# mll-lab-nu/TStar

Hardware: AMD Instinct MI355X
Metric: candidate frames scored/sec (whole node) + sec/video to 8 keyframes, 1h@1fps (higher is better)
Workload: dtype f32 held exactly as 3 bf16 terms per operand: every GEMM and vision-attention operand (activations, weights, Q, K, V, softmax probabilities) = three round-to-nearest bf16 terms carrying all 24 significand bits; the 6 partial products with i + j <= 2 (each exact) on v_mfma_f32_32x32x16_bf16, f32 accu

## Files before the change

include/tstar_hip.h:

```cpp
#ifndef TSTAR_HIP_H
#define TSTAR_HIP_H

#include <stddef.h>
#include <stdint.h>

#ifdef __cplusplus
extern "C" {
#endif

#define TSTAR_OK 0
#define TSTAR_ERR_ARG 1
#define TSTAR_ERR_HIP 2
#define TSTAR_ERR_STATE 3

#define TSTAR_OWL_NPATCH 576
#define TSTAR_OWL_QDIM 512
#define TSTAR_OWL_TEXT_LEN 16
#define TSTAR_OWL_MAX_QUERIES 32
#define TSTAR_OWL_MAX_SETS 64

const char* tstar_last_error(void);
int tstar_abi_version(void);
size_t tstar_owl_vision_blob_floats(void);
size_t tstar_owl_text_blob_floats(void);

typedef struct tstar_owl tstar_owl;

#define TSTAR_WEIGHTS_F32 0
#define TSTAR_WEIGHTS_BF16 1
#define TSTAR_WEIGHTS_BF16_EXACT 3
#define TSTAR_WEIGHTS_F32X3 4
int tstar_owl_create(tstar_owl** out, const float* h_vision_blob, size_t n_vision,
                     const float* h_text_blob, size_t n_text, const float* h_norm_lut, int max_batch,
                     int weights_mode);
int tstar_owl_create_ex(tstar_owl** out, int image_size, int patch_size, const float* h_vision_blob, size_t n_vision,
                        const float* h_text_blob, size_t n_text, const float* h_norm_lut, int max_batch, int weights_mode);
size_t tstar_owl_vision_blob_floats_ex(int image_size, int patch_size);
int tstar_owl_create_in(tstar_owl** out, int input_h, int input_w, int patch_size, const float* h_vision_blob, size_t n_vision,
                        const float* h_text_blob, size_t n_text, const float* h_norm_lut, int max_batch, int weights_mode);
size_t tstar_owl_vision_blob_floats_in(int input_h, int input_w, int patch_size);
#define TSTAR_OWL_FAMILY_OWLVIT 0
#define TSTAR_OWL_FAMILY_OWLV2 1
int tstar_owl_create_family(tstar_owl** out, int family, int input_h, int input_w, int patch_size, const float* h_vision_blob,
                            size_t n_vision, const float* h_text_blob, size_t n_text, const float* h_norm, int max_batch,
                            int weights_mode);
size_t tstar_owl_vision_blob_floats_family(int family, int input_h, int input_w, int patch_size);
int tstar_owl_num_patches(tstar_owl* h);
int tstar_owl_destroy(tstar_owl* h);

int tstar_owl_set_queries(tstar_owl* h, int query_set, const int32_t* h_input_ids, const int32_t* h_attention_mask,
                          const double* h_class_weight, int Q, void* stream);
int tstar_owl_set_queries_many(tstar_owl* h, int n_sets, const int32_t* h_sets, const int32_t* h_Q, const int32_t* h_ids,
                               const int32_t* h_am, const double* h_w, void* stream);
int tstar_owl_set_query_embeds(tstar_owl* h, int query_set, const float* h_query_embeds, const uint8_t* h_query_mask,
                               const double* h_class_weight, int Q, void* stream);
int tstar_owl_set_class_weights(tstar_owl* h, int query_set, const double* h_class_weight, int Q, void* stream);
int tstar_owl_get_query_embeds(tstar_owl* h, int query_set, float* h_out, int Q, void* stream);

int tstar_owl_score(tstar_owl* h, const uint8_t* d_images, int B, int H, int W, int grid_rows, int grid_cols,
                    const int32_t* h_image_query_set, float* d_scores, int32_t* d_labels, float* d_boxes_xyxy, double* d_cell_conf,
                    uint32_t* d_cell_mask, int32_t* d_n_kept, float* d_logits, float* d_boxes_cxcywh, void* stream);
#define TSTAR_OWL_LANES 2
#define TSTAR_OWL_AUX_BATCH 4
int tstar_owl_score_lane(tstar_owl* h, int lane, const uint8_t* d_images, int B, int H, int W, int grid_rows, int grid_cols,
                         const int32_t* h_image_query_set, float* d_scores, int32_t* d_labels, float* d_boxes_xyxy,
                         double* d_cell_conf, uint32_t* d_cell_mask, int32_t* d_n_kept, float* d_logits,
                         float* d_boxes_cxcywh, void* stream);

int tstar_owl_score_lane_obj(tstar_owl* h, int lane, const uint8_t* d_images, int B, int H, int W, int grid_rows, int grid_cols,
                             const int32_t* h_image_query_set, float* d_scores, int32_t* d_labels, float* d_boxes_xyxy,
                             double* d_cell_conf, uint32_t* d_cell_mask, int32_t* d_n_kept, float* d_logits,
                             float* d_boxes_cxcywh, float* d_objectness, void* stream);

int tstar_owlv2_set_axis_weights(tstar_owl* h, int S, int out, const double* gw, int n);
int tstar_owlv2_preprocess_plan(int H, int W, int out_h, int out_w, int* plan10);
int tstar_owlv2_axis_window(int S, int out, int tile, int k, int radius, int* lo_n2);
int tstar_owlv2_axis_tables(int S, int out, int32_t* i0, int32_t* i1, double* t, double* gw, int gw_cap);
int tstar_owlv2_last_preprocess_form(tstar_owl* h, int lane);

int tstar_owl_debug_preprocess(tstar_owl* h, const uint8_t* d_images, int B, int H, int W,
                               uint8_t* d_out_u8 , float* d_out_patches ,
                               void* stream);

int tstar_owl_debug_heads(tstar_owl* h, const float* d_feats, const float* d_cls, const float* d_boxh, int B, int H, int W,
                          const int32_t* h_image_query_set, float* d_scores, int32_t* d_labels, float* d_boxes_xyxy, float* d_logits,
                          float* d_boxes_cxcywh, const float* d_obj_hidden, float* d_objectness, void* stream);
int tstar_owl_debug_merge(tstar_owl* h, float* d_x, int B, int write_cls, float* d_feats, void* stream);
int tstar_owl_debug_embed(tstar_owl* h, const float* d_patches, int B, int stage, float* d_x, void* stream);
int tstar_owl_debug_text(tstar_owl* h, const int32_t* h_ids, const int32_t* h_am, int Q, int stage, float* h_out, void* stream);
int tstar_cell_reduce(const float* d_scores, const int32_t* d_labels, const float* d_boxes_xyxy, const double* h_weights, int n_sets,
                      const int32_t* h_image_set, int B, int np, int W, int H, int grid_rows, int grid_cols, float thr,
                      double* d_cell_conf, uint32_t* d_cell_mask, int32_t* d_n_kept, void* stream);

int tstar_owl_embed_image_queries(tstar_owl* h, const uint8_t* d_images, int n, int H, int W, float* h_embeds, int32_t* h_best,
                                  float* h_boxes_cxcywh, int32_t* h_n_selected, int32_t* h_status, void* stream);
int tstar_image_query_select(const float* d_cls, const float* d_boxes_cxcywh, int n, int np, float* h_embeds, int32_t* h_best,
                             float* h_boxes_cxcywh, int32_t* h_n_selected, int32_t* h_status, void* stream);

typedef struct tstar_yolo tstar_yolo;
int tstar_yolo_create(tstar_yolo** out, const float* h_blob, size_t n_blob, const int32_t* h_ops, int n_ops, int op_words,
                      const int32_t* h_bufs, int n_bufs, const int32_t* h_guides, int n_guides, const int32_t* h_levels,
                      int n_levels, int input_buf, int max_batch);
int tstar_yolo_destroy(tstar_yolo* h);
int tstar_yolo_num_anchors(tstar_yolo* h);
int tstar_yolo_set_text_feats(tstar_yolo* h, int query_set, const float* h_text, const double* h_class_weight, int Q, void* stream);
int tstar_yolo_set_class_weights(tstar_yolo* h, int query_set, const double* h_class_weight, int Q, void* stream);
int tstar_yolo_detect(tstar_yolo* h, const uint8_t* d_images, int B, int H, int W, int grid_rows, int grid_cols,
                      const int32_t* h_image_query_set, float score_threshold, int max_dets, float* d_det_scores,
                      int32_t* d_det_labels, float* d_det_boxes, int32_t* d_n_det, double* d_cell_conf, uint32_t* d_cell_mask,
                      float* d_dense_scores, float* d_dense_boxes, void* stream);
int tstar_yolo_postprocess(tstar_yolo* h, const float* const* d_level_embed, const float* const* d_level_dfl, int n_levels, int B, int H,
                           int W, int grid_rows, int grid_cols, const int32_t* h_image_query_set, float score_threshold, int max_dets,
                           float* d_det_scores, int32_t* d_det_labels, float* d_det_boxes, int32_t* d_n_det, double* d_cell_conf,
                           uint32_t* d_cell_mask, float* d_dense_scores, float* d_dense_boxes, void* stream);

#define TSTAR_YOLO_FORM_TILE64 0
#define TSTAR_YOLO_FORM_TILE128 1
#define TSTAR_YOLO_FORM_WIDE 2
#define TSTAR_YOLO_FORM_SW8 3
#define TSTAR_YOLO_FORM_SW4 4
#define TSTAR_YOLO_FORM_HALO_A16 5
#define TSTAR_YOLO_FORM_HALO_A8 6
#define TSTAR_YOLO_FORM_HALO_B16 7
#define TSTAR_YOLO_FORM_HALO_B8 8
#define TSTAR_YOLO_FORM_DIRECT 9
int tstar_yolo_buffer_copy(tstar_yolo* h, int buf, float* d_data, int B, int to_buffer, void* stream);
int tstar_yolo_run_ops(tstar_yolo* h, int B, const int32_t* h_image_query_set, int32_t* h_forms, void* stream);
int tstar_yolo_conv_plan(int cin, int src_ld, int src_off, int H, int W, int cout, int dst_ld, int dst_off, int ks, int stride, int mode, int B,
                         int max_batch, int env_policy, int* plan3);

int tstar_frames_to_grid(const uint8_t* d_video, int N, int H, int W, const int32_t* d_frame_idx,
                         int grid_rows, int grid_cols, uint8_t* d_grid, int nv12, void* stream);
int tstar_frames_resize(const uint8_t* d_video, int N, int H, int W, const int32_t* d_frame_idx, int n,
                        int out_w, int out_h, uint8_t* d_out, int nv12, void* stream);
int tstar_i420_to_nv12(const uint8_t* d_i420, int n, int H, int W, uint8_t* d_nv12, void* stream);
int tstar_jpeg_probe(const uint8_t* data, size_t len, int32_t* info5);
size_t tstar_jpeg_frame_end(const uint8_t* data, size_t len, size_t pos);
int tstar_jpeg_sizes(int W, int H, int ncomp, int hs, int vs, size_t* out2);
int tstar_jpeg_threads(int asked);
int tstar_jpeg_entropy_batch(const uint8_t* const* datas, const size_t* lens, int n, int W, int H, int ncomp, int hs, int vs,
                             int16_t* coef, uint16_t* quant, int threads, int32_t* status);
int tstar_jpeg_reconstruct_host(const int16_t* coef, const uint16_t* quant, int n, int W, int H, int ncomp, int hs, int vs,
                                uint8_t* rgb, int threads);
int tstar_jpeg_reconstruct(const int16_t* d_coef, const uint16_t* d_quant, int n, int W, int H, int ncomp, int hs, int vs,
                           uint8_t* d_planes, uint8_t* d_rgb, void* stream);
int tstar_nv12_to_rgb(const uint8_t* d_video, int N, int H, int W, const int32_t* d_frame_idx, int n,
                      uint8_t* d_out, void* stream);

typedef struct tstar_searcher tstar_searcher;
int tstar_searcher_create(tstar_searcher** out, int n_frames, double init_score, double init_p);
int tstar_searcher_destroy(tstar_searcher* s);
int tstar_searcher_apply_grid(tstar_searcher* s, const int32_t* h_secs, const double* d_conf, int n,
                              int* h_n_visited, int32_t* h_vis_x, double* h_vis_y, void* stream);
int tstar_searcher_window_spread(tstar_searcher* s, const int32_t* h_secs, const double* h_conf, int n, int window,
                                 void* stream);
int tstar_searcher_visited(tstar_searcher* s, int* h_n_visited, int32_t* h_vis_x, double* h_vis_y, void* stream);
int tstar_searcher_set_spline(tstar_searcher* s, const double* h_t, const double* h_c, int n_knots, int k, void* stream);
int tstar_searcher_sampler_prep(tstar_searcher* s, int num, double add, int* h_fallback, void* stream);
int tstar_searcher_pop_prep(tstar_searcher* s, int* h_nnz, double* h_sum, void* stream);
int tstar_searcher_draw(tstar_searcher* s, const double* h_x, int k, int32_t* h_idx, void* stream);
int tstar_searcher_exclude(tstar_searcher* s, const int32_t* h_found, int m, void* stream);
int tstar_searcher_set_scores(tstar_searcher* s, const int32_t* h_secs, const double* h_vals, int m, void* stream);
int tstar_searcher_read_state(tstar_searcher* s, double* h_out, void* stream);
int tstar_searcher_write(tstar_searcher* s, int which, const double* h_in, void* stream);
int tstar_searcher_read(tstar_searcher* s, int which, double* h_out, void* stream);

#define TSTAR_COMM_ID_BYTES 128
typedef struct tstar_comm tstar_comm;
int tstar_comm_available(void);
int tstar_comm_unique_id(void* h_id );
int tstar_comm_create(tstar_comm** out, const void* h_id, int world, int rank);
int tstar_comm_destroy(tstar_comm* c);
int tstar_allgather_i32(tstar_comm* c, const int32_t* d_send, int32_t* d_recv, int count, void* stream);

int tstar_topk_seconds(const double* d_P, int N, int clip_start, int clip_end, int k, int32_t* h_out, void* stream);

int tstar_ssim_pairwise(const uint8_t* d_gt, int G, const uint8_t* d_pred, int P, int H, int W,
                        const float* h_window, double* d_out, void* stream);

int tstar_draw_boxes(uint8_t* d_images, int B, int H, int W, const float* d_boxes_xyxy, const float* d_scores, void* stream);
int tstar_draw_boxes_np(uint8_t* d_images, int B, int H, int W, const float* d_boxes_xyxy, const float* d_scores, int np,
                        void* stream);

int tstar_gemm_f32(const float* d_A, const float* d_W, float* d_C, const float* d_bias, const float* d_residual,
                   int M, int N, int K, int act, void* stream);
int tstar_gemm_f32_cfg(const float* d_A, const float* d_W, float* d_C, const float* d_bias, const float* d_residual,
                       int M, int N, int K, int act, int tile_cfg, void* stream);
int tstar_gemm_bf16w(const float* d_A, const float* d_W, float* d_C, const float* d_bias, const float* d_residual,
                     int M, int N, int K, int act, int tile_cfg, void* stream);
int tstar_gemm_bf16w2(const float* d_A, const float* d_W, float* d_C, const float* d_bias, const float* d_residual,
                      int M, int N, int K, int act, int tile_cfg, void* stream);
int tstar_gemm_bf16w_pre(const float* d_A, const void* d_Wb, float* d_C, const float* d_bias, const float* d_residual,
                         int M, int N, int K, int act, int a_terms, int tile_cfg, void* stream);
int tstar_gemm_f32x3(const float* d_A, const float* d_W, float* d_C, const float* d_bias, const float* d_residual,
                     int M, int N, int K, int act, int tile_cfg, void* stream);
int tstar_pack_f32x3(const float* d_W, void* d_Wp, int N, int K, void* stream);
int tstar_gemm_f32x3_pre(const float* d_A, const void* d_Wp, float* d_C, const float* d_bias, const float* d_residual,
                         int M, int N, int K, int act, int tile_cfg, void* stream);
int tstar_gemm_plan(int weights_mode, int M, int N, int ldc, int patch_np, int tile_cfg, int has_packed_w2, int* plan4);
int tstar_gemm_patch_embed(const float* d_A, const float* d_W, float* d_X, const float* d_pos, int B, int np, int N, int K,
                           int weights_mode, int tile_cfg, void* stream);
int tstar_ingest_plan(int op, int nv12, int H, int W, int n, int ow, int oh, int out_aligned4, int video_aligned4, int generic,
                      int nv12_lds, int grid_px, int* plan6);
int tstar_layernorm_f32(const float* d_x, float* d_y, const float* d_w, const float* d_b, int rows, int D, void* stream);
int tstar_attention_f32(const float* d_qkv, float* d_out, int B, int T, int heads, int mode,
                        const uint8_t* d_key_mask, void* stream);

int tstar_attention_split(const float* d_qkv, float* d_out, int B, int T, int heads, void* stream);
int tstar_attention_x3(const float* d_qkv, float* d_out, int B, int T, int heads, void* stream);

int tstar_prof_enable(int on);
int tstar_prof_read(int category, long long* launches, double* total_ms, double* total_flops);
int tstar_prof_read_bytes(int category, double* total_bytes);
int tstar_prof_read_totals(int category, long long* launches_all, double* flops_all);
int tstar_prof_mark(int which, void* stream);

#ifdef __cplusplus
}
#endif
#endif
```

tstar_amd/_lib.py:

```python
from __future__ import annotations

import ctypes as C
import os

_HERE = os.path.dirname(os.path.abspath(__file__))
LIB_PATH = os.path.join(_HERE, "libtstar_hip.so")


class TStarHipError(RuntimeError):
    pass


_vp, _i, _sz = C.c_void_p, C.c_int, C.c_size_t
_fp = C.POINTER(C.c_float)
SIGNATURES = {
    "tstar_last_error": (C.c_char_p, []),
    "tstar_abi_version": (_i, []),
    "tstar_owl_vision_blob_floats": (_sz, []),
    "tstar_owl_text_blob_floats": (_sz, []),
    "tstar_owl_create": (_i, [C.POINTER(_vp), _vp, _sz, _vp, _sz, _vp, _i, _i]),
    "tstar_owl_create_ex": (_i, [C.POINTER(_vp), _i, _i, _vp, _sz, _vp, _sz, _vp, _i, _i]),
    "tstar_owl_vision_blob_floats_ex": (_sz, [_i, _i]),
    "tstar_owl_create_in": (_i, [C.POINTER(_vp), _i, _i, _i, _vp, _sz, _vp, _sz, _vp, _i, _i]),
    "tstar_owl_vision_blob_floats_in": (_sz, [_i, _i, _i]),
    "tstar_owl_create_family": (_i, [C.POINTER(_vp), _i, _i, _i, _i, _vp, _sz, _vp, _sz, _vp, _i, _i]),
    "tstar_owl_vision_blob_floats_family": (_sz, [_i, _i, _i, _i]),
    "tstar_owl_score_lane_obj": (_i, [_vp, _i, _vp, _i, _i, _i, _i, _i, _vp, _vp, _vp, _vp, _vp, _vp, _vp, _vp, _vp, _vp, _vp]),
    "tstar_owlv2_set_axis_weights": (_i, [_vp, _i, _i, _vp, _i]),
    "tstar_owlv2_preprocess_plan": (_i, [_i, _i, _i, _i, C.POINTER(_i)]),
    "tstar_owlv2_axis_window": (_i, [_i, _i, _i, _i, _i, C.POINTER(_i)]),
    "tstar_owlv2_axis_tables": (_i, [_i, _i, _vp, _vp, _vp, _vp, _i]),
    "tstar_owlv2_last_preprocess_form": (_i, [_vp, _i]),
    "tstar_owl_num_patches": (_i, [_vp]),
    "tstar_owl_destroy": (_i, [_vp]),
    "tstar_owl_set_queries": (_i, [_vp, _i, _vp, _vp, _vp, _i, _vp]),
    "tstar_owl_set_queries_many": (_i, [_vp, _i, _vp, _vp, _vp, _vp, _vp, _vp]),
    "tstar_owl_set_query_embeds": (_i, [_vp, _i, _vp, _vp, _vp, _i, _vp]),
    "tstar_owl_set_class_weights": (_i, [_vp, _i, _vp, _i, _vp]),
    "tstar_owl_get_query_embeds": (_i, [_vp, _i, _vp, _i, _vp]),
    "tstar_owl_score": (_i, [_vp, _vp, _i, _i, _i, _i, _i, _vp, _vp, _vp, _vp, _vp, _vp, _vp, _vp, _vp, _vp]),
    "tstar_owl_score_lane": (_i, [_vp, _i, _vp, _i, _i, _i, _i, _i, _vp, _vp, _vp, _vp, _vp, _vp, _vp, _vp, _vp, _vp]),
    "tstar_owl_debug_preprocess": (_i, [_vp, _vp, _i, _i, _i, _vp, _vp, _vp]),
    "tstar_owl_debug_heads": (_i, [_vp, _vp, _vp, _vp, _i, _i, _i, _vp, _vp, _vp, _vp, _vp, _vp, _vp, _vp, _vp]),
    "tstar_owl_debug_merge": (_i, [_vp, _vp, _i, _i, _vp, _vp]),
    "tstar_owl_debug_embed": (_i, [_vp, _vp, _i, _i, _vp, _vp]),
    "tstar_owl_debug_text": (_i, [_vp, _vp, _vp, _i, _i, _vp, _vp]),
    "tstar_cell_reduce": (_i, [_vp, _vp, _vp, _vp, _i, _vp, _i, _i, _i, _i, _i, _i, C.c_float, _vp, _vp, _vp, _vp]),
    "tstar_owl_embed_image_queries": (_i, [_vp, _vp, _i, _i, _i, _vp, _vp, _vp, _vp, _vp, _vp]),
    "tstar_image_query_select": (_i, [_vp, _vp, _i, _i, _vp, _vp, _vp, _vp, _vp, _vp]),
    "tstar_yolo_create": (_i, [C.POINTER(_vp), _vp, _sz, _vp, _i, _i, _vp, _i, _vp, _i, _vp, _i, _i, _i]),
    "tstar_yolo_destroy": (_i, [_vp]),
    "tstar_yolo_num_anchors": (_i, [_vp]),
    "tstar_yolo_set_text_feats": (_i, [_vp, _i, _vp, _vp, _i, _vp]),
    "tstar_yolo_set_class_weights": (_i, [_vp, _i, _vp, _i, _vp]),
    "tstar_yolo_detect": (_i, [_vp, _vp, _i, _i, _i, _i, _i, _vp, C.c_float, _i, _vp, _vp, _vp, _vp, _vp, _vp, _vp, _vp, _vp]),
    "tstar_yolo_postprocess": (_i, [_vp, _vp, _vp, _i, _i, _i, _i, _i, _i, _vp, C.c_float, _i, _vp, _vp, _vp, _vp, _vp, _vp, _vp, _vp, _vp]),
    "tstar_yolo_buffer_copy": (_i, [_vp, _i, _vp, _i, _i, _vp]),
    "tstar_yolo_run_ops": (_i, [_vp, _i, _vp, _vp, _vp]),
    "tstar_yolo_conv_plan": (_i, [_i] * 14 + [C.POINTER(_i)]),
    "tstar_frames_to_grid": (_i, [_vp, _i, _i, _i, _vp, _i, _i, _vp, _i, _vp]),
    "tstar_frames_resize": (_i, [_vp, _i, _i, _i, _vp, _i, _i, _i, _vp, _i, _vp]),
    "tstar_i420_to_nv12": (_i, [_vp, _i, _i, _i, _vp, _vp]),
    "tstar_nv12_to_rgb": (_i, [_vp, _i, _i, _i, _vp, _i, _vp, _vp]),
    "tstar_jpeg_probe": (_i, [_vp, _sz, _vp]),
    "tstar_jpeg_frame_end": (_sz, [_vp, _sz, _sz]),
    "tstar_jpeg_sizes": (_i, [_i, _i, _i, _i, _i, _vp]),
    "tstar_jpeg_threads": (_i, [_i]),
    "tstar_jpeg_entropy_batch": (_i, [_vp, _vp, _i, _i, _i, _i, _i, _i, _vp, _vp, _i, _vp]),
    "tstar_jpeg_reconstruct_host": (_i, [_vp, _vp, _i, _i, _i, _i, _i, _i, _vp, _i]),
    "tstar_jpeg_reconstruct": (_i, [_vp, _vp, _i, _i, _i, _i, _i, _i, _vp, _vp, _vp]),
    "tstar_searcher_create": (_i, [C.POINTER(_vp), _i, C.c_double, C.c_double]),
    "tstar_searcher_destroy": (_i, [_vp]),
    "tstar_searcher_apply_grid": (_i, [_vp, _vp, _vp, _i, _vp, _vp, _vp, _vp]),
    "tstar_searcher_set_spline": (_i, [_vp, _vp, _vp, _i, _i, _vp]),
    "tstar_searcher_sampler_prep": (_i, [_vp, _i, C.c_double, _vp, _vp]),
    "tstar_searcher_pop_prep": (_i, [_vp, _vp, _vp, _vp]),
    "tstar_searcher_window_spread": (_i, [_vp, _vp, _vp, _i, _i, _vp]),
    "tstar_searcher_visited": (_i, [_vp, _vp, _vp, _vp, _vp]),
    "tstar_searcher_write": (_i, [_vp, _i, _vp, _vp]),
    "tstar_searcher_draw": (_i, [_vp, _vp, _i, _vp, _vp]),
    "tstar_searcher_exclude": (_i, [_vp, _vp, _i, _vp]),
    "tstar_searcher_set_scores": (_i, [_vp, _vp, _vp, _i, _vp]),
    "tstar_searcher_read_state": (_i, [_vp, _vp, _vp]),
    "tstar_searcher_read": (_i, [_vp, _i, _vp, _vp]),
    "tstar_comm_available": (_i, []),
    "tstar_comm_unique_id": (_i, [_vp]),
    "tstar_comm_create": (_i, [C.POINTER(_vp), _vp, _i, _i]),
    "tstar_comm_destroy": (_i, [_vp]),
    "tstar_allgather_i32": (_i, [_vp, _vp, _vp, _i, _vp]),
    "tstar_topk_seconds": (_i, [_vp, _i, _i, _i, _i, _vp, _vp]),
    "tstar_ssim_pairwise": (_i, [_vp, _i, _vp, _i, _i, _i, _vp, _vp, _vp]),
    "tstar_gemm_f32": (_i, [_vp, _vp, _vp, _vp, _vp, _i, _i, _i, _i, _vp]),
    "tstar_gemm_f32_cfg": (_i, [_vp, _vp, _vp, _vp, _vp, _i, _i, _i, _i, _i, _vp]),
    "tstar_gemm_bf16w": (_i, [_vp, _vp, _vp, _vp, _vp, _i, _i, _i, _i, _i, _vp]),
    "tstar_gemm_bf16w2": (_i, [_vp, _vp, _vp, _vp, _vp, _i, _i, _i, _i, _i, _vp]),
    "tstar_gemm_bf16w_pre": (_i, [_vp, _vp, _vp, _vp, _vp, _i, _i, _i, _i, _i, _i, _vp]),
    "tstar_gemm_f32x3": (_i, [_vp, _vp, _vp, _vp, _vp, _i, _i, _i, _i, _i, _vp]),
    "tstar_pack_f32x3": (_i, [_vp, _vp, _i, _i, _vp]),
    "tstar_gemm_f32x3_pre": (_i, [_vp, _vp, _vp, _vp, _vp, _i, _i, _i, _i, _i, _vp]),
    "tstar_gemm_plan": (_i, [_i, _i, _i, _i, _i, _i, _i, C.POINTER(_i)]),
    "tstar_gemm_patch_embed": (_i, [_vp, _vp, _vp, _vp, _i, _i, _i, _i, _i, _i, _vp]),
    "tstar_ingest_plan": (_i, [_i] * 12 + [C.POINTER(_i)]),
    "tstar_layernorm_f32": (_i, [_vp, _vp, _vp, _vp, _i, _i, _vp]),
    "tstar_draw_boxes": (_i, [_vp, _i, _i, _i, _vp, _vp, _vp]),
    "tstar_draw_boxes_np": (_i, [_vp, _i, _i, _i, _vp, _vp, _i, _vp]),
    "tstar_attention_split": (_i, [_vp, _vp, _i, _i, _i, _vp]),
    "tstar_attention_x3": (_i, [_vp, _vp, _i, _i, _i, _vp]),
    "tstar_attention_f32": (_i, [_vp, _vp, _i, _i, _i, _i, _vp, _vp]),
    "tstar_prof_enable": (_i, [_i]),
    "tstar_prof_read": (_i, [_i, _vp, _vp, _vp]),
    "tstar_prof_read_bytes": (_i, [_i, _vp]),
    "tstar_prof_read_totals": (_i, [_i, _vp, _vp]),
    "tstar_prof_mark": (_i, [_i, _vp]),
}

_lib = None


def load() -> C.CDLL:
    global _lib
    if _lib is not None:
        return _lib
    if not os.path.isfile(LIB_PATH):
        raise TStarHipError(
            f"{LIB_PATH} is missing: build it with `python -m tstar_amd.build` "
            "(hipcc --offload-arch=gfx950). tstar_amd has no CPU fallback.")
    import torch
    lib = C.CDLL(LIB_PATH)
    for name, (res, args) in SIGNATURES.items():
        fn = getattr(lib, name)
        fn.restype = res
        fn.argtypes = args
    _lib = lib
    return lib


def check(rc: int, what: str = "") -> None:
    if rc != 0:
        msg = load().tstar_last_error()
        raise TStarHipError(f"{what or 'tstar_hip'} failed (code {rc}): {msg.decode() if msg else ''}")


def ptr(t) -> int:
    if t is None:
        return None
    if hasattr(t, "data_ptr"):
        return t.data_ptr()
    return t.ctypes.data


def stream_ptr():
    import torch
    return torch.cuda.current_stream().cuda_stream
```

tstar_amd/csrc/attention_x3.h:

```cpp
#pragma once
#include <hip/hip_runtime.h>
#include <math.h>
#include <utility>

namespace tstar {
namespace ax3 {

typedef __bf16 bf16x8 __attribute__((ext_vector_type(8)));
typedef __bf16 bf16x2 __attribute__((ext_vector_type(2)));
typedef float f32x2 __attribute__((ext_vector_type(2)));
typedef float f32x4 __attribute__((ext_vector_type(4)));
typedef float f32x16 __attribute__((ext_vector_type(16)));
typedef unsigned int u32x4 __attribute__((ext_vector_type(4)));
typedef unsigned int u32x2 __attribute__((ext_vector_type(2)));

constexpr int HD = 64, KB = 32;
constexpr int VPITCH = 80;
constexpr int KP = KB * 128, VP = HD * VPITCH;
constexpr int KBUF = 3 * KP, VBUF = 3 * VP, NKB = 2, NVB = 3;
constexpr int LDS_BYTES = NKB * KBUF + NVB * VBUF;

#define AX3_FENCE() __builtin_amdgcn_sched_barrier(0)

__device__ __forceinline__ void split2_rn3(float x0, float x1, unsigned (&o)[3]) {
#pragma unroll
    for (int k = 0; k < 3; ++k) {
        f32x2 x; x[0] = x0; x[1] = x1;
        const unsigned hb = __builtin_bit_cast(unsigned, __builtin_convertvector(x, bf16x2));
        o[k] = hb;
        if (k < 2) {
            x0 = x0 - __uint_as_float(hb << 16);
            x1 = x1 - __uint_as_float(hb & 0xFFFF0000u);
        }
    }
}
__device__ __forceinline__ float xhalf_max(float x) {
    const auto r = __builtin_amdgcn_permlane32_swap(__float_as_uint(x), __float_as_uint(x), false, false);
    return fmaxf(__uint_as_float(r[0]), __uint_as_float(r[1]));
}
__device__ __forceinline__ float xhalf_sum(float x) {
    const auto r = __builtin_amdgcn_permlane32_swap(__float_as_uint(x), __float_as_uint(x), false, false);
    return __uint_as_float(r[0]) + __uint_as_float(r[1]);
}

__device__ __forceinline__ int k_off(int key, int chunk) { return key * 128 + ((chunk ^ ((key >> 1) & 7)) << 4); }
__device__ __forceinline__ int v_off(int d, int chunk) { return d * VPITCH + (chunk << 4); }
__device__ __forceinline__ int v_keypos(int k) { const int g = k >> 2; const int gp = (g & 4) | ((g & 1) << 1) | ((g >> 1) & 1); return (gp * 4 + (k & 3)) * 2; }

__device__ __forceinline__ f32x16 mfma(const bf16x8 a, const u32x4 b, const f32x16 c) {
    return __builtin_amdgcn_mfma_f32_32x32x16_bf16(a, __builtin_bit_cast(bf16x8, b), c, 0, 0, 0);
}

template <bool PLANES>
__global__ __launch_bounds__(256, 2) void attention_x3_kernel(const float* __restrict__ qkv, const char* __restrict__ planes,
                                                              float* __restrict__ out, int T, int heads, int qtiles) {
    extern __shared__ __attribute__((aligned(16))) char smem[];
    char* const kbuf = smem;
    char* const vbuf = smem + NKB * KBUF;

    const int D = heads * HD, D3 = 3 * D;
    int bid = blockIdx.x;
    const int qt = bid % qtiles; bid /= qtiles;
    const int head = bid % heads;
    const int b = bid / heads;

    const int t = threadIdx.x, lane = t & 63, wave = __builtin_amdgcn_readfirstlane(t >> 6);
    const int l31 = lane & 31, h = lane >> 5;
    const size_t rowbase = (size_t)b * T;

    const int q = qt * 128 + wave * 32 + l31;
    const int qc = q < T ? q : T - 1;
    const bool wave_active = (qt * 128 + wave * 32) < T;

    u32x4 qp[3][4];
    {
        const float* src = qkv + (rowbase + qc) * D3 + head * HD + 8 * h;
        const float sc = 0.125f * 1.44269504088896340736f;
#pragma unroll
        for (int s = 0; s < 4; ++s) {
            const f32x4 a = *reinterpret_cast<const f32x4*>(src + 16 * s) * sc;
            const f32x4 c = *reinterpret_cast<const f32x4*>(src + 16 * s + 4) * sc;
            unsigned o0[3], o1[3], o2[3], o3[3];
            split2_rn3(a[0], a[1], o0); split2_rn3(a[2], a[3], o1); split2_rn3(c[0], c[1], o2); split2_rn3(c[2], c[3], o3);
#pragma unroll
            for (int k = 0; k < 3; ++k) { qp[k][s][0] = o0[k]; qp[k][s][1] = o1[k]; qp[k][s][2] = o2[k]; qp[k][s][3] = o3[k]; }
        }
    }

    const int kc4 = t & 15, kr = t >> 4;
    const int vkp = t & 15, vdq = t >> 4;
    const __amdgpu_buffer_rsrc_t kv_rsrc =
        __builtin_amdgcn_make_buffer_rsrc(const_cast<float*>(qkv + rowbase * D3), 0, (int)((size_t)T * D3 * 4), 0x00020000);
    int kvo[2], vvo[2];
#pragma unroll
    for (int i = 0; i < 2; ++i) {
        kvo[i] = ((kr + 16 * i) * D3 + D + head * HD + kc4 * 4) * 4;
        vvo[i] = ((2 * vkp + i) * D3 + 2 * D + head * HD + vdq * 4) * 4;
    }
    const int kwr0 = k_off(kr, kc4 >> 1) + (kc4 & 1) * 8, kwr1 = k_off(kr + 16, kc4 >> 1) + (kc4 & 1) * 8;
    int vwr[4];
#pragma unroll
    for (int e = 0; e < 4; ++e) {
        const int pos = v_keypos(2 * vkp);
        vwr[e] = v_off(4 * vdq + e, pos >> 4) + (pos & 15);
    }

    const int R0 = b * T;
    const int kt0 = R0 >> 5;
    const bool tail_key = !PLANES && (T % KB) == 1;
    const int nkb = PLANES ? ((R0 + T - 1) >> 5) - kt0 + 1 : (tail_key ? T / KB : (T + KB - 1) / KB);

    f32x4 rk[2], rv[2];
    auto gload = [&](int kb) __attribute__((always_inline)) {
        const int so = (kb < nkb ? kb : nkb) * (KB * 4) * D3;
#pragma unroll
        for (int i = 0; i < 2; ++i) {
            rk[i] = __builtin_bit_cast(f32x4, __builtin_amdgcn_raw_buffer_load_b128(kv_rsrc, kvo[i], so, 0));
            rv[i] = __builtin_bit_cast(f32x4, __builtin_amdgcn_raw_buffer_load_b128(kv_rsrc, vvo[i], so, 0));
        }
    };
    unsigned ksp[2][3];
    auto stage_piece = [&](auto P, char* kdst, char* vdst) __attribute__((always_inline)) {
        constexpr int p = decltype(P)::value;
        if constexpr (p < 4) {
            constexpr int i = p >> 1, hf = p & 1;
            split2_rn3(rk[i][2 * hf], rk[i][2 * hf + 1], ksp[hf]);
            if constexpr (hf == 1) {
#pragma unroll
                for (int k = 0; k < 3; ++k) {
                    u32x2 v; v[0] = ksp[0][k]; v[1] = ksp[1][k];
                    *reinterpret_cast<u32x2*>(kdst + k * KP + (i == 0 ? kwr0 : kwr1)) = v;
                }
            }
        } else {
            constexpr int e = p - 4;
            unsigned o[3];
            split2_rn3(rv[0][e], rv[1][e], o);
#pragma unroll
            for (int k = 0; k < 3; ++k) *reinterpret_cast<unsigned*>(vdst + k * VP + vwr[e]) = o[k];
        }
    };
    auto stage_all = [&](int kb) __attribute__((always_inline)) {
        char* kd = kbuf + (kb & 1) * KBUF;
        char* vd = vbuf + (kb % NVB) * VBUF;
// ... 250 lines not shown
            }
        }
        sx = xhalf_sum(sx);
        const float mn = fmaxf(m_run, sx);
        const float al = __builtin_amdgcn_exp2f(m_run - mn);
        const float p = __builtin_amdgcn_exp2f(sx - mn);
        l_run = l_run * al + p;
        m_run = mn;
#pragma unroll
        for (int g4 = 0; g4 < 4; ++g4) {
            const f32x4 v0 = *reinterpret_cast<const f32x4*>(qkv + ro + 2 * D + 8 * g4 + 4 * h);
            const f32x4 v1 = *reinterpret_cast<const f32x4*>(qkv + ro + 2 * D + 32 + 8 * g4 + 4 * h);
#pragma unroll
            for (int e = 0; e < 4; ++e) {
                o0[g4 * 4 + e] = o0[g4 * 4 + e] * al + p * v0[e];
                o1[g4 * 4 + e] = o1[g4 * 4 + e] * al + p * v1[e];
            }
        }
    }

    if (q < T) {
        const float inv = 1.0f / l_run;
        float* op = out + (rowbase + q) * D + head * HD + 4 * h;
#pragma unroll
        for (int g4 = 0; g4 < 4; ++g4) {
            f32x4 a, c;
#pragma unroll
            for (int e = 0; e < 4; ++e) { a[e] = o0[g4 * 4 + e] * inv; c[e] = o1[g4 * 4 + e] * inv; }
            *reinterpret_cast<f32x4*>(op + 8 * g4) = a;
            *reinterpret_cast<f32x4*>(op + 32 + 8 * g4) = c;
        }
    }
}

}

inline size_t kv_planes_bytes(int rows, int heads) { return (size_t)((rows + 31) / 32) * heads * (size_t)(ax3::KBUF + ax3::VBUF); }

#ifdef TSTAR_ATTN_X3_LAB
namespace ax3 {
__global__ __launch_bounds__(256) void kv_planes_kernel(const float* __restrict__ qkv, char* __restrict__ planes, int rows, int heads) {
    const int D = heads * HD, D3 = 3 * D;
    const size_t gid = (size_t)blockIdx.x * 256 + threadIdx.x;
    const int dq = (int)(gid % 16), head = (int)((gid / 16) % heads);
    const size_t rp = gid / (16 * (size_t)heads);
    const int row = (int)(rp * 2);
    if (row >= ((rows + 31) / 32) * 32) return;
    const int kt = row >> 5, key = row & 31;
    char* tile = planes + ((size_t)kt * heads + head) * (size_t)(KBUF + VBUF);
    f32x4 kx[2], vx[2];
#pragma unroll
    for (int i = 0; i < 2; ++i) {
        if (row + i < rows) {
            kx[i] = *reinterpret_cast<const f32x4*>(qkv + (size_t)(row + i) * D3 + D + head * HD + dq * 4);
            vx[i] = *reinterpret_cast<const f32x4*>(qkv + (size_t)(row + i) * D3 + 2 * D + head * HD + dq * 4);
        } else {
            kx[i] = f32x4{0.f, 0.f, 0.f, 0.f};
            vx[i] = f32x4{0.f, 0.f, 0.f, 0.f};
        }
    }
#pragma unroll
    for (int i = 0; i < 2; ++i) {
        unsigned o0[3], o1[3];
        split2_rn3(kx[i][0], kx[i][1], o0);
        split2_rn3(kx[i][2], kx[i][3], o1);
#pragma unroll
        for (int k = 0; k < 3; ++k) {
            u32x2 v; v[0] = o0[k]; v[1] = o1[k];
            *reinterpret_cast<u32x2*>(tile + k * KP + k_off(key + i, dq >> 1) + (dq & 1) * 8) = v;
        }
    }
    const int pos = v_keypos(key);
#pragma unroll
    for (int e = 0; e < 4; ++e) {
        unsigned o[3];
        split2_rn3(vx[0][e], vx[1][e], o);
#pragma unroll
        for (int k = 0; k < 3; ++k) *reinterpret_cast<unsigned*>(tile + KBUF + k * VP + v_off(4 * dq + e, pos >> 4) + (pos & 15)) = o[k];
    }
}
}
#endif

inline int attention_x3_launch(const float* qkv, float* out, int B, int T, int heads, hipStream_t s, const char* planes = nullptr) {
    const int qtiles = (T + 127) / 128;
#ifdef TSTAR_ATTN_X3_LAB
    static bool attr[2] = {false, false};
    if (planes) {
        if (!attr[1]) {
            const hipError_t e = hipFuncSetAttribute(reinterpret_cast<const void*>(ax3::attention_x3_kernel<true>), hipFuncAttributeMaxDynamicSharedMemorySize, ax3::LDS_BYTES);
            if (e != hipSuccess) return (int)e;
            attr[1] = true;
        }
        hipLaunchKernelGGL(ax3::attention_x3_kernel<true>, dim3(B * heads * qtiles), dim3(256), ax3::LDS_BYTES, s, qkv, planes, out, T, heads, qtiles);
        return (int)hipGetLastError();
    }
    if (!attr[0]) {
        const hipError_t e = hipFuncSetAttribute(reinterpret_cast<const void*>(ax3::attention_x3_kernel<false>), hipFuncAttributeMaxDynamicSharedMemorySize, ax3::LDS_BYTES);
        if (e != hipSuccess) return (int)e;
        attr[0] = true;
    }
#endif
    if (planes) return (int)hipErrorInvalidValue;
    hipLaunchKernelGGL(ax3::attention_x3_kernel<false>, dim3(B * heads * qtiles), dim3(256), ax3::LDS_BYTES, s, qkv, planes, out, T, heads, qtiles);
    return (int)hipGetLastError();
}

#ifdef TSTAR_ATTN_X3_LAB
inline int kv_planes_launch(const float* qkv, char* planes, int rows, int heads, hipStream_t s) {
    const size_t n = (size_t)((rows + 31) / 32) * 16 * 16 * heads;
    hipLaunchKernelGGL(ax3::kv_planes_kernel, dim3((unsigned)((n + 255) / 256)), dim3(256), 0, s, qkv, planes, rows, heads);
    return (int)hipGetLastError();
}
#endif

}
```

tstar_amd/csrc/attention_x3.hip:

```cpp
#include "common.h"
#include "kernels.h"
#include "prof.h"
#include "attention_x3.h"

namespace tstar {

int attention_x3(const float* qkv, float* out, int B, int T, int heads, hipStream_t s) {
    TSTAR_REQUIRE(B > 0 && T > 0 && heads > 0, "attention_x3: empty problem");
    TSTAR_REQUIRE(((size_t)T + 32) * 3 * heads * 64 * 4 < (1ull << 31), "attention_x3: one image's qkv rows (plus one key tile of look-ahead) must stay below 2 GiB");
    if (int rc = ensure_dyn_lds(reinterpret_cast<const void*>(ax3::attention_x3_kernel<false>), ax3::LDS_BYTES)) return rc;
    const bool prof = prof_enabled();
    if (prof) prof_start(PROF_ATTN, s, 4.0 * B * heads * (double)T * T * 64);
    const int rc = attention_x3_launch(qkv, out, B, T, heads, s);
    if (prof) prof_stop(PROF_ATTN, s);
    TSTAR_HIP_CHECK((hipError_t)rc);
    return TSTAR_OK;
}

}
```

tstar_amd/csrc/capi.hip:

```cpp
#include "../../include/tstar_hip.h"
#include "common.h"
#include "heads.h"
#include "image_query.h"
#include "ingest.h"
#include "jpeg_host.h"
#include "kernels.h"
#include "owl_weights.h"
#include "preprocess_v2.h"
#include <math.h>
#include <map>
#include <mutex>
#include <set>
#include <string.h>
#include <unordered_map>
#include <vector>

namespace tstar {
static thread_local std::string g_err;
void set_error(const std::string& msg) { g_err = msg; }

int ensure_dyn_lds(const void* kernel, int bytes) {
    static std::mutex mu;
    static std::set<std::pair<const void*, int>> done;
    int dev = 0;
// ... 230 lines not shown
static int preprocess_chunk(tstar_owl* h, tstar_owl::Lane& L, const uint8_t* d_images, int B, int H, int W, uint8_t* out_u8,
                            float* out_patches, hipStream_t s) {
    if (h->geom.family == TSTAR_OWL_FAMILY_OWLV2) {
        TSTAR_REQUIRE(!out_u8, "tstar_owl_debug_preprocess: an OWLv2 handle has no u8 stage (d_out_u8 must be NULL)");
        return preprocess_chunk_v2(h, L, d_images, B, H, W, out_patches, s);
    }
    ResampleTable *th, *tv;
    const OwlGeom& G = h->geom;
    RC(get_table(h, W, G.in_w, &th, s));
    RC(get_table(h, H, G.in_h, &tv, s));
    const size_t need = (size_t)B * H * G.in_w * 3;
    if (need > L.tmp_u8_bytes) {
        TSTAR_HIP_CHECK(hipStreamSynchronize(s));
        if (L.tmp_u8) TSTAR_HIP_CHECK(hipFree(L.tmp_u8));
        L.tmp_u8 = nullptr; L.tmp_u8_bytes = 0;
        TSTAR_HIP_CHECK(hipMalloc(&L.tmp_u8, need));
        L.tmp_u8_bytes = need;
    }
    RC(resample_h_u8(d_images, L.tmp_u8, B, H, W, *th, s));
    RC(resample_v_normalize_patchify(L.tmp_u8, out_patches, out_u8, B, H, G.in_w, *tv, h->d_lut, G.patch, s));
    return TSTAR_OK;
}

static hipError_t alloc_lane(tstar_owl::Lane& L, int cap, const OwlGeom& g) {
    const size_t mp = lane_rows(cap, g);
    hipError_t e = hipSuccess;
    auto alloc = [&](float** p, size_t n) { if (e == hipSuccess) { e = hipMalloc(p, n * sizeof(float)); if (e == hipSuccess) e = hipMemset(*p, 0, n * sizeof(float)); } };
    alloc(&L.x, mp * V_D); alloc(&L.xn, mp * V_D); alloc(&L.qkv, mp * 3 * V_D); alloc(&L.att, mp * V_D); alloc(&L.hid, mp * V_FF);
    if (e == hipSuccess) L.cap = cap;
    return e;
}
static void free_lane(tstar_owl::Lane& L) {
    void* ptrs[] = {L.x, L.xn, L.qkv, L.att, L.hid, L.tmp_u8, L.d_image_set, L.d_minmax};
    for (void* p : ptrs) if (p) (void)hipFree(p);
    L = tstar_owl::Lane{};
}

#define CHECK_SET(set, fn) TSTAR_REQUIRE((set) >= 0 && (set) < TSTAR_OWL_MAX_SETS, fn ": query_set must be in 0..63")

static int check_image_sets(const tstar_owl* h, const int32_t* h_image_query_set, int B, int* q_uniform) {
    int qu = -1;
    for (int b = 0; b < B; ++b) {
        const int set = h_image_query_set ? h_image_query_set[b] : 0;
        CHECK_SET(set, "tstar_owl_score");
        if (h->Q[set] == 0) { set_error("tstar_owl_score: no queries installed in the requested query set (call tstar_owl_set_queries first)"); return TSTAR_ERR_STATE; }
        qu = (b == 0 || qu == h->Q[set]) ? h->Q[set] : 0;
    }
    *q_uniform = qu;
    return TSTAR_OK;
}

static int stage_image_sets(tstar_owl::Lane& L, const int32_t* h_image_query_set, int B, hipStream_t s) {
    if (B > L.image_set_cap) {
        TSTAR_HIP_CHECK(hipStreamSynchronize(s));
        if (L.d_image_set) TSTAR_HIP_CHECK(hipFree(L.d_image_set));
        L.d_image_set = nullptr; L.image_set_cap = 0;
        TSTAR_HIP_CHECK(hipMalloc(&L.d_image_set, (size_t)B * sizeof(int)));
        L.image_set_cap = B;
    }
    TSTAR_HIP_CHECK(hipMemcpyAsync(L.d_image_set, h_image_query_set, (size_t)B * sizeof(int), hipMemcpyHostToDevice, s));
    return TSTAR_OK;
}

static void box_scale(const OwlGeom& G, int H, int W, float* sx, float* sy) {
    const bool v2 = G.family == TSTAR_OWL_FAMILY_OWLV2;
    *sx = (float)(v2 ? (H > W ? H : W) : W);
    *sy = (float)(v2 ? (H > W ? H : W) : H);
}

static DetectRowsArgs detect_args(const tstar_owl* h) {
    DetectRowsArgs a{};
    a.qn = h->qn; a.qmask = h->qmask; a.setQ = h->d_setQ;
    a.shift_w = h->vw.shift_w; a.shift_b = h->vw.shift_b; a.scale_w = h->vw.scale_w; a.scale_b = h->vw.scale_b;
    a.box2_w = h->vw.box2_w; a.box2_b = h->vw.box2_b; a.box_bias = h->vw.box_bias;
    return a;
}

struct OwlHeadTensors {
    float* feats;
    float* cls;
    float* bh1;
    float* bh2;
};
static int owl_forward_heads(tstar_owl* h, tstar_owl::Lane& L, const uint8_t* d_images, int Bc, int H, int W, OwlHeadTensors* t, hipStream_t s) {
    const OwlGeom& G = h->geom;
    const int NP = G.np, NTOK = G.ntok, PK = G.patch_k;
    const int M = Bc * NTOK, MP = Bc * NP;
    RC(preprocess_chunk(h, L, d_images, Bc, H, W, nullptr, L.hid, s));
    GemmArgs pg = mk_gemm(h, L.hid, h->vw.patch_w, L.x, nullptr, nullptr, MP, V_D, PK, PK, V_D, ACT_NONE);
    pg.pos = h->vw.pos_emb; pg.patch_np = NP;
    RC(gemm_f32(pg, s));
    RC(write_cls_rows(L.x, h->vw.class_emb, h->vw.pos_emb, Bc, NTOK, V_D, s));
    RC(layernorm_f32(L.x, L.x, h->vw.pre_ln_w, h->vw.pre_ln_b, M, V_D, s));
    RC(run_encoder(h, L, h->vw.layers, V_LAYERS, Bc, NTOK, V_D, V_FF, V_HEADS, 0, nullptr, s));
    t->feats = L.xn; t->cls = L.att; t->bh1 = L.qkv; t->bh2 = L.hid;
    RC(merge_cls_ln(L.x, t->feats, h->vw.post_ln_w, h->vw.post_ln_b, h->vw.det_ln_w, h->vw.det_ln_b, Bc, NTOK, V_D, s));
    RC(gemm_f32(mk_gemm(h, t->feats, h->vw.cls_w, t->cls, h->vw.cls_b, nullptr, MP, PROJ, V_D, V_D, PROJ, ACT_NONE), s));
    RC(gemm_f32(mk_gemm(h, t->feats, h->vw.box0_w, t->bh1, h->vw.box0_b, nullptr, MP, V_D, V_D, V_D, V_D, ACT_GELU), s));
    RC(gemm_f32(mk_gemm(h, t->bh1, h->vw.box1_w, t->bh2, h->vw.box1_b, nullptr, MP, V_D, V_D, V_D, V_D, ACT_GELU), s));
    return TSTAR_OK;
}

extern "C" {

const char* tstar_last_error(void) { return g_err.c_str(); }
int tstar_abi_version(void) { return 3; }
size_t tstar_owl_vision_blob_floats(void) { return vision_floats(OwlGeom{}); }
size_t tstar_owl_text_blob_floats(void) { return text_floats(); }
size_t tstar_owl_vision_blob_floats_ex(int image_size, int patch_size) {
    OwlGeom g;
    if (!owl_geom(image_size, patch_size, &g)) { set_error("tstar_owl_vision_blob_floats_ex: unsupported geometry (image 768, patch 32 or 16)"); return 0; }
    return vision_floats(g);
}
size_t tstar_owl_vision_blob_floats_in(int input_h, int input_w, int patch_size) {
    OwlGeom g;
    if (!owl_geom_input(input_h, input_w, patch_size, &g)) {
        set_error("tstar_owl_vision_blob_floats_in: unsupported input size (patch 32 or 16; each side a positive multiple of the patch size; at most 3600 patches)");
        return 0;
    }
    return vision_floats(g);
}
size_t tstar_owl_vision_blob_floats_family(int family, int input_h, int input_w, int patch_size) {
    OwlGeom g;
    if (!owl_geom_family(family, input_h, input_w, patch_size, &g)) {
        set_error("tstar_owl_vision_blob_floats_family: unsupported family / input size (family 0: patch 32 or 16; family 1 (OWLv2): patch 16; each "
                  "side a positive multiple of the patch size; at most 3600 patches)");
        return 0;
    }
    return vision_floats(g);
}
int tstar_owl_num_patches(tstar_owl* h) {
    if (!h) { set_error("tstar_owl_num_patches: null handle"); return -1; }
    return h->geom.np;
}

static int make_bf16_copies(tstar_owl* h, int mode) {
    struct Mat { const float* w; int n, k; };
    std::vector<Mat> mats;
    mats.push_back({h->vw.patch_w, V_D, h->geom.patch_k});
    auto layer = [&](const LayerW& l, int d, int ff) {
        mats.push_back({l.qkv_w, 3 * d, d}); mats.push_back({l.out_w, d, d});
        mats.push_back({l.fc1_w, ff, d}); mats.push_back({l.fc2_w, d, ff});
    };
    for (int i = 0; i < V_LAYERS; ++i) layer(h->vw.layers[i], V_D, V_FF);
    mats.push_back({h->vw.cls_w, PROJ, V_D});
    mats.push_back({h->vw.box0_w, V_D, V_D});
    mats.push_back({h->vw.box1_w, V_D, V_D});
    if (h->vw.obj0_w) { mats.push_back({h->vw.obj0_w, V_D, V_D}); mats.push_back({h->vw.obj1_w, V_D, V_D}); }
    if (h->has_text) {
        for (int i = 0; i < T_LAYERS; ++i) layer(h->tw.layers[i], T_D, T_FF);
        mats.push_back({h->tw.text_proj, PROJ, T_D});
    }
    for (auto& m : mats) {
        const size_t n = (size_t)m.n * m.k;
        int rc;
        if (mode == TSTAR_WEIGHTS_F32X3) {
            void* p = nullptr;
            TSTAR_HIP_CHECK(hipMalloc(&p, n * 6));
            h->wp[m.w] = p;
            rc = pack_weights_x3(m.w, p, m.n, m.k, 0);
        } else {
            __bf16* p = nullptr;
            TSTAR_HIP_CHECK(hipMalloc(&p, n * sizeof(__bf16)));
            h->wb[m.w] = p;
            rc = convert_f32_to_bf16(m.w, p, nullptr, n, 0);
            static const bool w2v_off = getenv("TSTAR_W2V_OFF") != nullptr;
            if (!rc && mode == TSTAR_WEIGHTS_BF16 && m.n == 768 && m.k % 32 == 0 && !w2v_off) {
                void* q = nullptr;
                TSTAR_HIP_CHECK(hipMalloc(&q, n * sizeof(__bf16)));
                h->wq[m.w] = q;
                rc = pack_weights_w2(p, q, m.n, m.k, 0);
            }
        }
        if (rc) return rc;
    }
    TSTAR_HIP_CHECK(hipDeviceSynchronize());
    h->weights_mode = mode;
    return TSTAR_OK;
}

// ... 209 lines not shown
        TSTAR_HIP_CHECK(hipMalloc(&h->d_kmask, (size_t)cap * T_LEN));
        h->seq_cap = cap;
    }
    std::vector<int> eos(total);
    std::vector<uint8_t> km((size_t)total * T_LEN), qm(total);
    for (int q = 0; q < total; ++q) {
        int best = 0;
        for (int t = 0; t < T_LEN; ++t) {
            if (h_ids[q * T_LEN + t] > h_ids[q * T_LEN + best]) best = t;
            km[(size_t)q * T_LEN + t] = h_am[q * T_LEN + t] != 0;
        }
        eos[q] = best;
        qm[q] = h_ids[q * T_LEN] > 0;
    }
    int i0 = 0, q0 = 0;
    while (i0 < n_sets) {
        int i1 = i0, nseq = 0;
        while (i1 < n_sets && nseq + h_Q[i1] <= cap) nseq += h_Q[i1++];
        const int M = nseq * T_LEN;
        TSTAR_HIP_CHECK(hipMemcpyAsync(h->d_ids, h_ids + (size_t)q0 * T_LEN, (size_t)M * sizeof(int), hipMemcpyHostToDevice, s));
        TSTAR_HIP_CHECK(hipMemcpyAsync(h->d_eos, eos.data() + q0, nseq * sizeof(int), hipMemcpyHostToDevice, s));
        TSTAR_HIP_CHECK(hipMemcpyAsync(h->d_kmask, km.data() + (size_t)q0 * T_LEN, M, hipMemcpyHostToDevice, s));
        hipLaunchKernelGGL(embed_tokens_kernel, dim3(M), dim3(128), 0, s, h->d_ids, h->tw.tok_emb, h->tw.tpos_emb, L.x, T_LEN, T_D);
        TSTAR_HIP_CHECK(hipGetLastError());
        RC(run_encoder(h, L, h->tw.layers, T_LAYERS, nseq, T_LEN, T_D, T_FF, T_HEADS, 1, h->d_kmask, s));
        RC(layernorm_f32(L.x, L.xn, h->tw.final_ln_w, h->tw.final_ln_b, M, T_D, s));
        hipLaunchKernelGGL(gather_rows_kernel, dim3(nseq), dim3(128), 0, s, L.xn, h->d_eos, L.att, T_LEN, T_D);
        TSTAR_HIP_CHECK(hipGetLastError());
        RC(gemm_f32(mk_text_gemm(h, L.att, h->tw.text_proj, L.hid, nullptr, nullptr, nseq, PROJ, T_D, T_D, PROJ, ACT_NONE), s));
        int off = 0;
        for (int i = i0; i < i1; ++i) {
            const int set = h_sets[i], Q = h_Q[i];
            const size_t qo = (size_t)set * TSTAR_OWL_MAX_QUERIES;
            hipLaunchKernelGGL(l2norm_rows_kernel, dim3(Q), dim3(64), 0, s, L.hid + (size_t)off * PROJ, h->q_raw + qo * PROJ, 0.0f);
            hipLaunchKernelGGL(l2norm_rows_kernel, dim3(Q), dim3(64), 0, s, h->q_raw + qo * PROJ, h->qn + qo * PROJ, 1e-6f);
            TSTAR_HIP_CHECK(hipGetLastError());
            TSTAR_HIP_CHECK(hipMemcpyAsync(h->qmask + qo, qm.data() + q0 + off, Q, hipMemcpyHostToDevice, s));
            TSTAR_HIP_CHECK(hipMemcpyAsync(h->qweight + qo, h_w + q0 + off, Q * sizeof(double), hipMemcpyHostToDevice, s));
            h->Q[set] = Q;
            off += Q;
        }
        TSTAR_HIP_CHECK(hipStreamSynchronize(s));
        q0 += nseq;
        i0 = i1;
    }
    TSTAR_HIP_CHECK(hipMemcpyAsync(h->d_setQ, h->Q, sizeof(h->Q), hipMemcpyHostToDevice, s));
    TSTAR_HIP_CHECK(hipStreamSynchronize(s));
    return TSTAR_OK;
}

int tstar_owl_set_query_embeds(tstar_owl* h, int query_set, const float* h_qe, const uint8_t* h_mask, const double* h_w,
                               int Q, void* stream) {
    TSTAR_REQUIRE(h && h_qe && h_mask && h_w, "tstar_owl_set_query_embeds: null argument");
    CHECK_SET(query_set, "tstar_owl_set_query_embeds");
    TSTAR_REQUIRE(Q >= 1 && Q <= TSTAR_OWL_MAX_QUERIES, "tstar_owl_set_query_embeds: Q must be in 1..32");
    hipStream_t s = (hipStream_t)stream;
    TSTAR_HIP_CHECK(hipMemcpyAsync(h->q_raw + (size_t)query_set * TSTAR_OWL_MAX_QUERIES * PROJ, h_qe,
                                   (size_t)Q * PROJ * sizeof(float), hipMemcpyHostToDevice, s));
    return finish_queries(h, query_set, h_mask, h_w, Q, s);
}

int tstar_owl_set_class_weights(tstar_owl* h, int query_set, const double* h_w, int Q, void* stream) {
    TSTAR_REQUIRE(h && h_w, "tstar_owl_set_class_weights: null argument");
    CHECK_SET(query_set, "tstar_owl_set_class_weights");
    TSTAR_REQUIRE(Q == h->Q[query_set] && Q >= 1, "tstar_owl_set_class_weights: Q does not match the installed queries");
    hipStream_t s = (hipStream_t)stream;
    TSTAR_HIP_CHECK(hipMemcpyAsync(h->qweight + (size_t)query_set * TSTAR_OWL_MAX_QUERIES, h_w, Q * sizeof(double),
                                   hipMemcpyHostToDevice, s));
    TSTAR_HIP_CHECK(hipStreamSynchronize(s));
    return TSTAR_OK;
}

int tstar_owl_get_query_embeds(tstar_owl* h, int query_set, float* h_out, int Q, void* stream) {
    TSTAR_REQUIRE(h && h_out, "tstar_owl_get_query_embeds: null argument");
    CHECK_SET(query_set, "tstar_owl_get_query_embeds");
    TSTAR_REQUIRE(Q == h->Q[query_set], "tstar_owl_get_query_embeds: Q does not match the installed queries");
    hipStream_t s = (hipStream_t)stream;
    TSTAR_HIP_CHECK(hipMemcpyAsync(h_out, h->q_raw + (size_t)query_set * TSTAR_OWL_MAX_QUERIES * PROJ,
                                   (size_t)Q * PROJ * sizeof(float), hipMemcpyDeviceToHost, s));
    TSTAR_HIP_CHECK(hipStreamSynchronize(s));
    return TSTAR_OK;
}

int tstar_owl_score(tstar_owl* h, const uint8_t* d_images, int B, int H, int W, int grid_rows, int grid_cols,
                    const int32_t* h_image_query_set, float* d_scores, int32_t* d_labels, float* d_boxes_xyxy, double* d_cell_conf,
                    uint32_t* d_cell_mask, int32_t* d_n_kept, float* d_logits, float* d_boxes_cxcywh, void* stream) {
    return tstar_owl_score_lane(h, 0, d_images, B, H, W, grid_rows, grid_cols, h_image_query_set, d_scores, d_labels, d_boxes_xyxy, d_cell_conf,
                                d_cell_mask, d_n_kept, d_logits, d_boxes_cxcywh, stream);
}

int tstar_owl_score_lane(tstar_owl* h, int lane, const uint8_t* d_images, int B, int H, int W, int grid_rows, int grid_cols,
                         const int32_t* h_image_query_set, float* d_scores, int32_t* d_labels, float* d_boxes_xyxy, double* d_cell_conf,
                         uint32_t* d_cell_mask, int32_t* d_n_kept, float* d_logits, float* d_boxes_cxcywh, void* stream) {
    return tstar_owl_score_lane_obj(h, lane, d_images, B, H, W, grid_rows, grid_cols, h_image_query_set, d_scores, d_labels, d_boxes_xyxy, d_cell_conf,
                                    d_cell_mask, d_n_kept, d_logits, d_boxes_cxcywh, nullptr, stream);
}

int tstar_owl_score_lane_obj(tstar_owl* h, int lane, const uint8_t* d_images, int B, int H, int W, int grid_rows, int grid_cols,
                             const int32_t* h_image_query_set, float* d_scores, int32_t* d_labels, float* d_boxes_xyxy, double* d_cell_conf,
                             uint32_t* d_cell_mask, int32_t* d_n_kept, float* d_logits, float* d_boxes_cxcywh, float* d_objectness, void* stream) {
    TSTAR_REQUIRE(h && d_images && d_scores && d_labels && d_boxes_xyxy && d_cell_conf && d_cell_mask,
                  "tstar_owl_score: null argument");
    TSTAR_REQUIRE(lane >= 0 && lane < TSTAR_OWL_LANES, "tstar_owl_score_lane: lane must be 0 or 1");
    TSTAR_REQUIRE(B >= 1 && H >= 1 && W >= 1, "tstar_owl_score: empty batch or image");
    TSTAR_REQUIRE(grid_rows >= 1 && grid_cols >= 1, "tstar_owl_score: grid must be at least 1x1");
    if (!h->has_vision) { set_error("tstar_owl_score: handle was created without vision weights (text-only)"); return TSTAR_ERR_STATE; }
    TSTAR_REQUIRE(!d_objectness || h->geom.family == TSTAR_OWL_FAMILY_OWLV2, "tstar_owl_score_lane_obj: objectness needs an OWLv2 handle (OWL-ViT has no objectness head)");
    if (h->geom.family == TSTAR_OWL_FAMILY_OWLV2) {
        const Owlv2Plan vp = plan_owlv2_preprocess(H, W, h->geom.in_h, h->geom.in_w);
        if (vp.error) { set_error(vp.error); return TSTAR_ERR_ARG; }
    }
    hipStream_t s = (hipStream_t)stream;
    auto& L = h->lane[lane];
    if (lane != 0) {
        int need = B > TSTAR_OWL_AUX_BATCH ? B : TSTAR_OWL_AUX_BATCH;
        if (need > h->chunk_cap) need = h->chunk_cap;
        if (!L.x || L.cap < need) {
            if (L.x) { TSTAR_HIP_CHECK(hipDeviceSynchronize()); free_lane(L); }
            const hipError_t e = alloc_lane(L, need, h->geom);
            if (e != hipSuccess) {
                free_lane(L);
                set_error(std::string("tstar_owl_score_lane: workspace allocation failed: ") + hipGetErrorString(e));
                return TSTAR_ERR_HIP;
            }
            TSTAR_HIP_CHECK(hipDeviceSynchronize());
        }
    }
    int q_uniform = -1;
    RC(check_image_sets(h, h_image_query_set, B, &q_uniform));
    TSTAR_REQUIRE(!d_logits || q_uniform > 0, "tstar_owl_score: raw logits need the same query count for every image");
    if (h_image_query_set) RC(stage_image_sets(L, h_image_query_set, B, s));
    const int ncell = grid_rows * grid_cols;
    const OwlGeom& G = h->geom;
    const int NP = G.np;
    for (int b0 = 0; b0 < B; b0 += L.cap) {
        const int Bc = (B - b0) < L.cap ? (B - b0) : L.cap;
        const int MP = Bc * NP;
        OwlHeadTensors t;
        RC(owl_forward_heads(h, L, d_images + (size_t)b0 * H * W * 3, Bc, H, W, &t, s));
        float *feats = t.feats, *cls = t.cls, *bh1 = t.bh1, *bh2 = t.bh2;
        DetectRowsArgs a = detect_args(h);
        a.feats = feats; a.cls = cls; a.boxh = bh2;
        a.scores = d_scores + (size_t)b0 * NP;
        a.labels = d_labels + (size_t)b0 * NP;
        a.xyxy = d_boxes_xyxy + (size_t)b0 * NP * 4;
        a.logits = d_logits ? d_logits + (size_t)b0 * NP * q_uniform : nullptr;
        a.image_set = h_image_query_set ? L.d_image_set + b0 : nullptr;
        a.cxcywh = d_boxes_cxcywh ? d_boxes_cxcywh + (size_t)b0 * NP * 4 : nullptr;
        a.rows = MP; a.np = NP; a.Q = q_uniform;
        box_scale(G, H, W, &a.box_sx, &a.box_sy);
        RC(detect_rows(a, s));
        if (d_objectness) {
            RC(gemm_f32(mk_gemm(h, feats, h->vw.obj0_w, bh1, h->vw.obj0_b, nullptr, MP, V_D, V_D, V_D, V_D, ACT_GELU), s));
            RC(gemm_f32(mk_gemm(h, bh1, h->vw.obj1_w, bh2, h->vw.obj1_b, nullptr, MP, V_D, V_D, V_D, V_D, ACT_GELU), s));
            RC(row_dot768(bh2, h->vw.obj2_w, h->vw.obj2_b, d_objectness + (size_t)b0 * NP, MP, s));
        }
        RC(cell_reduce(a.scores, a.labels, a.xyxy, h->qweight, a.image_set, Bc, NP, W, H, grid_rows, grid_cols, 0.005f,
                       d_cell_conf + (size_t)b0 * ncell, d_cell_mask + (size_t)b0 * ncell,
                       d_n_kept ? d_n_kept + b0 : nullptr, s));
    }
    return TSTAR_OK;
}

int tstar_owl_debug_preprocess(tstar_owl* h, const uint8_t* d_images, int B, int H, int W, uint8_t* d_out_u8,
                               float* d_out_patches, void* stream) {
    TSTAR_REQUIRE(h && d_images && d_out_patches, "tstar_owl_debug_preprocess: null argument");
    TSTAR_REQUIRE(B >= 1 && B <= h->max_batch, "tstar_owl_debug_preprocess: B must be in 1..max_batch");
    if (!h->has_vision) { set_error("tstar_owl_debug_preprocess: handle was created without vision weights (text-only)"); return TSTAR_ERR_STATE; }
    return preprocess_chunk(h, h->lane[0], d_images, B, H, W, d_out_u8, d_out_patches, (hipStream_t)stream);
}

int tstar_owl_debug_heads(tstar_owl* h, const float* d_feats, const float* d_cls, const float* d_boxh, int B, int H, int W,
                          const int32_t* h_image_query_set, float* d_scores, int32_t* d_labels, float* d_boxes_xyxy, float* d_logits,
                          float* d_boxes_cxcywh, const float* d_obj_hidden, float* d_objectness, void* stream) {
    TSTAR_REQUIRE(h && d_feats && d_cls && d_boxh && d_scores && d_labels && d_boxes_xyxy, "tstar_owl_debug_heads: null argument");
    TSTAR_REQUIRE(B >= 1 && B <= h->max_batch, "tstar_owl_debug_heads: B must be in 1..max_batch");
    TSTAR_REQUIRE(H >= 1 && W >= 1, "tstar_owl_debug_heads: empty image");
    if (!h->has_vision) { set_error("tstar_owl_debug_heads: handle was created without vision weights (text-only)"); return TSTAR_ERR_STATE; }
    TSTAR_REQUIRE(!d_obj_hidden == !d_objectness, "tstar_owl_debug_heads: d_obj_hidden and d_objectness go together");
    TSTAR_REQUIRE(!d_objectness || h->geom.family == TSTAR_OWL_FAMILY_OWLV2, "tstar_owl_debug_heads: objectness needs an OWLv2 handle (OWL-ViT has no objectness head)");
    hipStream_t s = (hipStream_t)stream;
    auto& L = h->lane[0];
    int q_uniform = -1;
    RC(check_image_sets(h, h_image_query_set, B, &q_uniform));
    TSTAR_REQUIRE(!d_logits || q_uniform > 0, "tstar_owl_debug_heads: raw logits need the same query count for every image");
    if (h_image_query_set) RC(stage_image_sets(L, h_image_query_set, B, s));
    const int NP = h->geom.np;
    DetectRowsArgs a = detect_args(h);
    a.feats = d_feats; a.cls = d_cls; a.boxh = d_boxh;
    a.scores = d_scores; a.labels = d_labels; a.xyxy = d_boxes_xyxy; a.logits = d_logits; a.cxcywh = d_boxes_cxcywh;
    a.image_set = h_image_query_set ? L.d_image_set : nullptr;
    a.rows = B * NP; a.np = NP; a.Q = q_uniform;
    box_scale(h->geom, H, W, &a.box_sx, &a.box_sy);
    RC(detect_rows(a, s));
    if (d_objectness) RC(row_dot768(d_obj_hidden, h->vw.obj2_w, h->vw.obj2_b, d_objectness, B * NP, s));
    return TSTAR_OK;
}

int tstar_owl_debug_merge(tstar_owl* h, float* d_x, int B, int write_cls, float* d_feats, void* stream) {
    TSTAR_REQUIRE(h && d_x && d_feats, "tstar_owl_debug_merge: null argument");
    TSTAR_REQUIRE(B >= 1 && B <= h->max_batch, "tstar_owl_debug_merge: B must be in 1..max_batch");
    if (!h->has_vision) { set_error("tstar_owl_debug_merge: handle was created without vision weights (text-only)"); return TSTAR_ERR_STATE; }
    hipStream_t s = (hipStream_t)stream;
    if (write_cls) RC(write_cls_rows(d_x, h->vw.class_emb, h->vw.pos_emb, B, h->geom.ntok, V_D, s));
    return merge_cls_ln(d_x, d_feats, h->vw.post_ln_w, h->vw.post_ln_b, h->vw.det_ln_w, h->vw.det_ln_b, B, h->geom.ntok, V_D, s);
}

int tstar_owl_debug_embed(tstar_owl* h, const float* d_patches, int B, int stage, float* d_x, void* stream) {
    TSTAR_REQUIRE(h && d_patches && d_x, "tstar_owl_debug_embed: null argument");
    TSTAR_REQUIRE(stage == 0 || stage == 1, "tstar_owl_debug_embed: stage must be 0 (patch GEMM + class rows) or 1 (+ pre-LayerNorm)");
    if (!h->has_vision) { set_error("tstar_owl_debug_embed: handle was created without vision weights (text-only)"); return TSTAR_ERR_STATE; }
    auto& L = h->lane[0];
    TSTAR_REQUIRE(B >= 1 && B <= L.cap, "tstar_owl_debug_embed: B must be in 1..the images of one forward chunk (min(max_batch, chunk limit))");
    hipStream_t s = (hipStream_t)stream;
    const OwlGeom& G = h->geom;
    const int M = B * G.ntok;
    GemmArgs pg = mk_gemm(h, d_patches, h->vw.patch_w, L.x, nullptr, nullptr, B * G.np, V_D, G.patch_k, G.patch_k, V_D, ACT_NONE);
    pg.pos = h->vw.pos_emb; pg.patch_np = G.np;
    RC(gemm_f32(pg, s));
    RC(write_cls_rows(L.x, h->vw.class_emb, h->vw.pos_emb, B, G.ntok, V_D, s));
    if (stage == 1) RC(layernorm_f32(L.x, L.x, h->vw.pre_ln_w, h->vw.pre_ln_b, M, V_D, s));
    TSTAR_HIP_CHECK(hipMemcpyAsync(d_x, L.x, (size_t)M * V_D * sizeof(float), hipMemcpyDeviceToDevice, s));
    return TSTAR_OK;
}

int tstar_cell_reduce(const float* d_scores, const int32_t* d_labels, const float* d_boxes_xyxy, const double* h_weights, int n_sets,
                      const int32_t* h_image_set, int B, int np, int W, int H, int grid_rows, int grid_cols, float thr,
                      double* d_cell_conf, uint32_t* d_cell_mask, int32_t* d_n_kept, void* stream) {
    TSTAR_REQUIRE(d_scores && d_labels && d_boxes_xyxy && h_weights && d_cell_conf && d_cell_mask && d_n_kept, "tstar_cell_reduce: null argument");
    TSTAR_REQUIRE(B >= 1 && np >= 1 && W >= 1 && H >= 1, "tstar_cell_reduce: empty batch or image");
    TSTAR_REQUIRE(n_sets >= 1 && n_sets <= TSTAR_OWL_MAX_SETS, "tstar_cell_reduce: n_sets must be in 1..64");
    TSTAR_REQUIRE(grid_rows > 0 && grid_cols > 0 && grid_rows * grid_cols <= 4096, "tstar_cell_reduce: grid must have 1..4096 cells");
    for (int b = 0; h_image_set && b < B; ++b)
        TSTAR_REQUIRE(h_image_set[b] >= 0 && h_image_set[b] < n_sets, "tstar_cell_reduce: image set out of range");
    hipStream_t s = (hipStream_t)stream;
    double* d_w = nullptr;
    int* d_set = nullptr;
    TSTAR_HIP_CHECK(hipMalloc(&d_w, (size_t)n_sets * TSTAR_OWL_MAX_QUERIES * sizeof(double)));
    hipError_t e = hipMemcpyAsync(d_w, h_weights, (size_t)n_sets * TSTAR_OWL_MAX_QUERIES * sizeof(double), hipMemcpyHostToDevice, s);
    if (e == hipSuccess && h_image_set) {
        e = hipMalloc(&d_set, (size_t)B * sizeof(int));
        if (e == hipSuccess) e = hipMemcpyAsync(d_set, h_image_set, (size_t)B * sizeof(int), hipMemcpyHostToDevice, s);
    }
    int rc = TSTAR_OK;
    if (e == hipSuccess)
        rc = cell_reduce(d_scores, d_labels, d_boxes_xyxy, d_w, d_set, B, np, W, H, grid_rows, grid_cols, thr, d_cell_conf, d_cell_mask, d_n_kept, s);
    if (e == hipSuccess) e = hipStreamSynchronize(s);
    (void)hipFree(d_w);
    if (d_set) (void)hipFree(d_set);
    if (!rc && e != hipSuccess) { set_error(std::string("tstar_cell_reduce: ") + hipGetErrorString(e)); rc = TSTAR_ERR_HIP; }
    return rc;
}

static int image_query_finish(const char* fn, int rc, void* d_buf, const ImageQueryOut& o, int n, float* h_embeds, int32_t* h_best, float* h_boxes,
                              int32_t* h_n_selected, int32_t* h_status, hipStream_t s) {
    hipError_t e = hipSuccess;
    if (!rc) {
        e = hipMemcpyAsync(h_embeds, o.embeds, (size_t)n * 512 * sizeof(float), hipMemcpyDeviceToHost, s);
        if (e == hipSuccess) e = hipMemcpyAsync(h_boxes, o.boxes, (size_t)n * 4 * sizeof(float), hipMemcpyDeviceToHost, s);
        if (e == hipSuccess) e = hipMemcpyAsync(h_best, o.best, (size_t)n * sizeof(int), hipMemcpyDeviceToHost, s);
        if (e == hipSuccess) e = hipMemcpyAsync(h_n_selected, o.n_selected, (size_t)n * sizeof(int), hipMemcpyDeviceToHost, s);
        if (e == hipSuccess) e = hipMemcpyAsync(h_status, o.status, (size_t)n * sizeof(int), hipMemcpyDeviceToHost, s);
    }
    const hipError_t e2 = hipStreamSynchronize(s);
    if (e == hipSuccess) e = e2;
    (void)hipFree(d_buf);
    if (!rc && e != hipSuccess) { set_error(std::string(fn) + ": " + hipGetErrorString(e)); rc = TSTAR_ERR_HIP; }
    return rc;
}

int tstar_image_query_select(const float* d_cls, const float* d_boxes_cxcywh, int n, int np, float* h_embeds, int32_t* h_best, float* h_boxes_cxcywh,
                             int32_t* h_n_selected, int32_t* h_status, void* stream) {
    TSTAR_REQUIRE(d_cls && d_boxes_cxcywh && h_embeds && h_best && h_boxes_cxcywh && h_n_selected && h_status, "tstar_image_query_select: null argument");
    TSTAR_REQUIRE(n >= 1 && n <= 65535, "tstar_image_query_select: n must be in 1..65535");
    TSTAR_REQUIRE(np >= 1 && np <= IMAGE_QUERY_MAX_NP, "tstar_image_query_select: np must be in 1..3600");
    TSTAR_REQUIRE(((uintptr_t)d_cls & 15) == 0, "tstar_image_query_select: d_cls must be 16-byte aligned");
    hipStream_t s = (hipStream_t)stream;
    void* d_buf = nullptr;
    TSTAR_HIP_CHECK(hipMalloc(&d_buf, image_query_out_bytes(n)));
    const ImageQueryOut o = image_query_out_at(d_buf, n);
    const int rc = image_query_select(d_cls, d_boxes_cxcywh, n, np, o, s);
    return image_query_finish("tstar_image_query_select", rc, d_buf, o, n, h_embeds, h_best, h_boxes_cxcywh, h_n_selected, h_status, s);
}

int tstar_owl_embed_image_queries(tstar_owl* h, const uint8_t* d_images, int n, int H, int W, float* h_embeds, int32_t* h_best, float* h_boxes_cxcywh,
                                  int32_t* h_n_selected, int32_t* h_status, void* stream) {
    TSTAR_REQUIRE(h && d_images && h_embeds && h_best && h_boxes_cxcywh && h_n_selected && h_status, "tstar_owl_embed_image_queries: null argument");
    TSTAR_REQUIRE(n >= 1 && n <= 65535 && H >= 1 && W >= 1, "tstar_owl_embed_image_queries: empty batch or image (n in 1..65535)");
    if (!h->has_vision) { set_error("tstar_owl_embed_image_queries: handle was created without vision weights (text-only)"); return TSTAR_ERR_STATE; }
    if (h->geom.family == TSTAR_OWL_FAMILY_OWLV2) {
        const Owlv2Plan vp = plan_owlv2_preprocess(H, W, h->geom.in_h, h->geom.in_w);
        if (vp.error) { set_error(vp.error); return TSTAR_ERR_ARG; }
    }
    hipStream_t s = (hipStream_t)stream;
    auto& L = h->lane[0];
    const int NP = h->geom.np;
    void* d_buf = nullptr;
    TSTAR_HIP_CHECK(hipMalloc(&d_buf, image_query_out_bytes(n)));
    const ImageQueryOut o = image_query_out_at(d_buf, n);
    int rc = TSTAR_OK;
    for (int b0 = 0; b0 < n && !rc; b0 += L.cap) {
        const int Bc = (n - b0) < L.cap ? (n - b0) : L.cap;
        const int MP = Bc * NP;
        OwlHeadTensors t;
        rc = owl_forward_heads(h, L, d_images + (size_t)b0 * H * W * 3, Bc, H, W, &t, s);
        if (rc) break;
        const size_t R = round_up((size_t)MP, 4);
        DetectRowsArgs a = detect_args(h);
        a.feats = t.feats; a.cls = t.cls; a.boxh = t.bh2;
        a.scores = L.x; a.labels = reinterpret_cast<int*>(L.x + R); a.xyxy = L.x + 2 * R; a.cxcywh = L.x + 6 * R;
        a.logits = nullptr; a.image_set = nullptr;
        a.rows = MP; a.np = NP; a.Q = h->Q[0];
        box_scale(h->geom, H, W, &a.box_sx, &a.box_sy);
        rc = detect_rows(a, s);
        if (!rc) rc = image_query_select(t.cls, a.cxcywh, Bc, NP, image_query_out_offset(o, b0), s);
    }
    return image_query_finish("tstar_owl_embed_image_queries", rc, d_buf, o, n, h_embeds, h_best, h_boxes_cxcywh, h_n_selected, h_status, s);
}

int tstar_owlv2_last_preprocess_form(tstar_owl* h, int lane) {
    if (!h || lane < 0 || lane >= TSTAR_OWL_LANES) { set_error("tstar_owlv2_last_preprocess_form: null handle or bad lane"); return -1; }
    return h->lane[lane].v2_form;
}

int tstar_owlv2_set_axis_weights(tstar_owl* h, int S, int out, const double* gw, int n) {
    TSTAR_REQUIRE(h && gw && S >= 2 && out >= 1, "tstar_owlv2_set_axis_weights: bad argument");
    const Owlv2Axis a = owlv2_axis(S, out);
    TSTAR_REQUIRE(n == (a.radius > 0 ? a.radius : 0) + 1, "tstar_owlv2_set_axis_weights: n must be the axis' radius + 1");
    const auto key = std::make_pair(S, out);
    auto it = h->tabs_v2.find(key);
    if (it != h->tabs_v2.end()) {
        TSTAR_HIP_CHECK(hipDeviceSynchronize());
        free_owlv2_axis_table(&it->second);
        h->tabs_v2.erase(it);
    }
    h->gw_v2[key] = std::vector<double>(gw, gw + n);
    return TSTAR_OK;
}

int tstar_owlv2_preprocess_plan(int H, int W, int out_h, int out_w, int* plan10) {
    TSTAR_REQUIRE(plan10, "tstar_owlv2_preprocess_plan: null argument");
    const Owlv2Plan p = plan_owlv2_preprocess(H, W, out_h, out_w);
    if (p.error) { set_error(p.error); return TSTAR_ERR_ARG; }
    const int v[10] = {p.form, p.tile_h, p.tile_w, p.win_h, p.win_w, p.lds_bytes, p.grid_x, p.grid_y, p.radius_y, p.radius_x};
    for (int i = 0; i < 10; ++i) plan10[i] = v[i];
    return TSTAR_OK;
}

int tstar_owlv2_axis_window(int S, int out, int tile, int k, int radius, int* lo_n2) {
    TSTAR_REQUIRE(lo_n2 && S >= 2 && out >= 1 && tile >= 1 && k >= 0 && k * tile < out, "tstar_owlv2_axis_window: bad argument");
    owlv2_axis_window(S, out, tile, k, radius, &lo_n2[0], &lo_n2[1]);
    return TSTAR_OK;
}

int tstar_owlv2_axis_tables(int S, int out, int32_t* i0, int32_t* i1, double* t, double* gw, int gw_cap) {
    TSTAR_REQUIRE(i0 && i1 && t && gw && S >= 2 && out >= 1, "tstar_owlv2_axis_tables: bad argument");
    std::vector<int> a, b;
    std::vector<double> tt, g;
    owlv2_axis_host(S, out, a, b, tt, g);
    TSTAR_REQUIRE((int)g.size() <= gw_cap, "tstar_owlv2_axis_tables: gw_cap is smaller than radius + 1");
    for (int j = 0; j < out; ++j) { i0[j] = a[j]; i1[j] = b[j]; t[j] = tt[j]; }
    for (size_t k = 0; k < g.size(); ++k) gw[k] = g[k];
    return TSTAR_OK;
}

int tstar_frames_to_grid(const uint8_t* d_video, int N, int H, int W, const int32_t* d_frame_idx, int grid_rows,
                         int grid_cols, uint8_t* d_grid, int nv12, void* stream) {
    TSTAR_REQUIRE(d_video && d_frame_idx && d_grid, "tstar_frames_to_grid: null argument");
    TSTAR_REQUIRE(N >= 1 && H >= 2 && W >= 2, "tstar_frames_to_grid: bad video shape");
    TSTAR_REQUIRE(!nv12 || (H % 2 == 0 && W % 2 == 0), "tstar_frames_to_grid: NV12 needs even dimensions");
    return frames_to_grid_u8(d_video, H, W, d_frame_idx, grid_rows, grid_cols, 200, 95, d_grid, nv12, (hipStream_t)stream);
}

int tstar_frames_resize(const uint8_t* d_video, int N, int H, int W, const int32_t* d_frame_idx, int n, int out_w,
                        int out_h, uint8_t* d_out, int nv12, void* stream) {
    TSTAR_REQUIRE(d_video && d_frame_idx && d_out, "tstar_frames_resize: null argument");
    TSTAR_REQUIRE(N >= 1 && H >= 2 && W >= 2, "tstar_frames_resize: bad video shape");
    TSTAR_REQUIRE(!nv12 || (H % 2 == 0 && W % 2 == 0), "tstar_frames_resize: NV12 needs even dimensions");
    return bilinear_gather_u8(d_video, H, W, d_frame_idx, n, out_w, out_h, d_out, nv12, (hipStream_t)stream);
}

int tstar_nv12_to_rgb(const uint8_t* d_video, int N, int H, int W, const int32_t* d_frame_idx, int n, uint8_t* d_out,
                      void* stream) {
    TSTAR_REQUIRE(d_video && d_frame_idx && d_out, "tstar_nv12_to_rgb: null argument");
    TSTAR_REQUIRE(N >= 1 && H >= 2 && W >= 2, "tstar_nv12_to_rgb: bad video shape");
    return nv12_to_rgb_u8(d_video, H, W, d_frame_idx, n, d_out, (hipStream_t)stream);
}

// ... 121 lines not shown
    return TSTAR_OK;
}

int tstar_gemm_patch_embed(const float* d_A, const float* d_W, float* d_X, const float* d_pos, int B, int np, int N, int K,
                           int weights_mode, int tile_cfg, void* stream) {
    TSTAR_REQUIRE(d_A && d_W && d_X && d_pos, "tstar_gemm_patch_embed: null argument");
    TSTAR_REQUIRE(B >= 1 && np >= 1, "tstar_gemm_patch_embed: B and np must be at least 1");
    TSTAR_REQUIRE((long long)B * (np + 1ll) < (1ll << 31), "tstar_gemm_patch_embed: B * (np + 1) token rows do not fit an int");
    const int wmode = gemm_wmode_of(weights_mode);
    TSTAR_REQUIRE(wmode >= 0, "tstar_gemm_patch_embed: unknown weights_mode (a TSTAR_WEIGHTS_* value)");
    TSTAR_REQUIRE(N > 0 && K > 0 && K % 32 == 0, "tstar_gemm_patch_embed: K must be a positive multiple of 32 (gemm_f32)");
    const int M = B * np;
    const bool two_term = weights_mode == TSTAR_WEIGHTS_BF16;
    const bool has_wq = two_term && N % 256 == 0;
    const GemmPlan p = plan_gemm(wmode, M, N, N, np, tile_cfg, has_wq);
    if (p.error) { set_error(std::string("tstar_gemm_patch_embed: ") + p.error); return TSTAR_ERR_ARG; }
    hipStream_t s = (hipStream_t)stream;
    __bf16* wb = nullptr;
    void *wq = nullptr, *wp = nullptr;
    int rc = TSTAR_OK;
    if (two_term || weights_mode == TSTAR_WEIGHTS_BF16_EXACT) {
        TSTAR_HIP_CHECK(hipMalloc(&wb, (size_t)N * K * sizeof(__bf16)));
        rc = convert_f32_to_bf16(d_W, wb, nullptr, (size_t)N * K, s);
        if (!rc && has_wq) {
            TSTAR_HIP_CHECK(hipMalloc(&wq, (size_t)N * K * sizeof(__bf16)));
            rc = pack_weights_w2(wb, wq, N, K, s);
        }
    } else if (weights_mode == TSTAR_WEIGHTS_F32X3) {
        TSTAR_HIP_CHECK(hipMalloc(&wp, (size_t)N * K * 6));
        rc = pack_weights_x3(d_W, wp, N, K, s);
    }
    if (!rc) {
        GemmArgs g = mk_gemm(nullptr, d_A, d_W, d_X, nullptr, nullptr, M, N, K, K, N, ACT_NONE);
        g.Wb = wb; g.Wq = wq; g.Wp = wp;
        g.a_terms = two_term ? 2 : wb ? 3 : 0;
        g.pos = d_pos; g.patch_np = np;
        g.tile_cfg = tile_cfg;
        rc = gemm_f32(g, s);
    }
    hipError_t e = hipStreamSynchronize(s);
    if (wb) (void)hipFree(wb);
    if (wq) (void)hipFree(wq);
    if (wp) (void)hipFree(wp);
    if (!rc && e != hipSuccess) { set_error(std::string("tstar_gemm_patch_embed: ") + hipGetErrorString(e)); rc = TSTAR_ERR_HIP; }
    return rc;
}

int tstar_ingest_plan(int op, int nv12, int H, int W, int n, int ow, int oh, int out_aligned4, int video_aligned4, int generic, int nv12_lds,
                      int grid_px, int* plan6) {
    TSTAR_REQUIRE(plan6, "tstar_ingest_plan: null argument");
    const IngestPlan p = plan_ingest(op, nv12 != 0, H, W, n, ow, oh, out_aligned4 != 0, video_aligned4 != 0, IngestOverrides{generic != 0, nv12_lds != 0, grid_px});
    if (p.error) { set_error(p.error); return TSTAR_ERR_ARG; }
    plan6[0] = p.kind; plan6[1] = p.px; plan6[2] = (int)p.grid_x; plan6[3] = (int)p.grid_y; plan6[4] = p.lds_bytes; plan6[5] = p.lds_pitch;
    return TSTAR_OK;
}

int tstar_layernorm_f32(const float* d_x, float* d_y, const float* d_w, const float* d_b, int rows, int D, void* stream) {
    TSTAR_REQUIRE(d_x && d_y && d_w && d_b, "tstar_layernorm_f32: null argument");
    return layernorm_f32(d_x, d_y, d_w, d_b, rows, D, (hipStream_t)stream);
}

int tstar_attention_f32(const float* d_qkv, float* d_out, int B, int T, int heads, int mode, const uint8_t* d_key_mask,
                        void* stream) {
    TSTAR_REQUIRE(d_qkv && d_out, "tstar_attention_f32: null argument");
    return attention_f32(d_qkv, d_out, B, T, heads, mode, d_key_mask, (hipStream_t)stream);
}

int tstar_draw_boxes(uint8_t* d_images, int B, int H, int W, const float* d_boxes_xyxy, const float* d_scores, void* stream) {
    TSTAR_REQUIRE(d_images && d_boxes_xyxy && d_scores, "tstar_draw_boxes: null argument");
    return draw_boxes(d_images, B, H, W, d_boxes_xyxy, d_scores, V_NP, 0.005f, (hipStream_t)stream);
}

int tstar_draw_boxes_np(uint8_t* d_images, int B, int H, int W, const float* d_boxes_xyxy, const float* d_scores, int np, void* stream) {
    TSTAR_REQUIRE(d_images && d_boxes_xyxy && d_scores, "tstar_draw_boxes_np: null argument");
    TSTAR_REQUIRE(np >= 1, "tstar_draw_boxes_np: np must be positive");
    return draw_boxes(d_images, B, H, W, d_boxes_xyxy, d_scores, np, 0.005f, (hipStream_t)stream);
}

int tstar_attention_x3(const float* d_qkv, float* d_out, int B, int T, int heads, void* stream) {
    TSTAR_REQUIRE(d_qkv && d_out, "tstar_attention_x3: null argument");
    return attention_x3(d_qkv, d_out, B, T, heads, (hipStream_t)stream);
}

int tstar_attention_split(const float* d_qkv, float* d_out, int B, int T, int heads, void* stream) {
    TSTAR_REQUIRE(d_qkv && d_out, "tstar_attention_split: null argument");
    return attention_split(d_qkv, d_out, B, T, heads, (hipStream_t)stream);
}

}
```

tstar_amd/csrc/common.h:

```cpp
#pragma once
#include <hip/hip_runtime.h>
#include <stdint.h>
#include <stdio.h>
#include <string>

namespace tstar {

void set_error(const std::string& msg);

#define TSTAR_HIP_CHECK(expr)                                                        \
    do {                                                                             \
        hipError_t _e = (expr);                                                      \
        if (_e != hipSuccess) {                                                      \
            ::tstar::set_error(std::string(#expr) + ": " + hipGetErrorString(_e));   \
            return TSTAR_ERR_HIP;                                                    \
        }                                                                            \
    } while (0)

#define TSTAR_REQUIRE(cond, msg)                                                     \
    do {                                                                             \
        if (!(cond)) {                                                               \
            ::tstar::set_error(std::string(msg) + " (" #cond ")");                  \
            return TSTAR_ERR_ARG;                                                    \
        }                                                                            \
    } while (0)

int ensure_dyn_lds(const void* kernel, int bytes);

static inline int cdiv(int a, int b) { return (a + b - 1) / b; }
static inline size_t round_up(size_t a, size_t b) { return (a + b - 1) / b * b; }

typedef float f32x4 __attribute__((ext_vector_type(4)));
typedef float f32x16 __attribute__((ext_vector_type(16)));

__device__ __forceinline__ int xcd_remap(int bid, int nwg) {
    const int nx = 8;
    int xcd = bid % nx, idx = bid / nx;
    int q = nwg / nx, r = nwg % nx;
    int base = (xcd < r) ? xcd * (q + 1) : r * (q + 1) + (xcd - r) * q;
    return base + idx;
}

__device__ __forceinline__ void store_px4(uint8_t* d, const unsigned (&v)[4][3]) {
    uint3 o;
    o.x = v[0][0] | (v[0][1] << 8) | (v[0][2] << 16) | (v[1][0] << 24);
    o.y = v[1][1] | (v[1][2] << 8) | (v[2][0] << 16) | (v[2][1] << 24);
    o.z = v[2][2] | (v[3][0] << 8) | (v[3][1] << 16) | (v[3][2] << 24);
    *reinterpret_cast<uint3*>(d) = o;
}

__device__ __forceinline__ double np_floor_divide(double a, double b) {
    const double mod = fmod(a, b);
    const double div = (a - mod) / b;
    const double f = floor(div);
    return div - f > 0.5 ? f + 1.0 : f;
}

}

#define TSTAR_OK 0
#define TSTAR_ERR_ARG 1
#define TSTAR_ERR_HIP 2
#define TSTAR_ERR_STATE 3
```

tstar_amd/csrc/heads.hip:

```cpp
#include "common.h"
#include "kernels.h"
#include "heads.h"
#include <float.h>

namespace tstar {

__device__ __forceinline__ float wsum(float v) {
#pragma unroll
    for (int o = 32; o > 0; o >>= 1) v += __shfl_xor(v, o);
    return v;
}

__global__ __launch_bounds__(256) void detect_rows_kernel(DetectRowsArgs a) {
    const int lane = threadIdx.x & 63;
    const int row = blockIdx.x * 4 + (threadIdx.x >> 6);
    if (row >= a.rows) return;
    const int p = row % a.np;

    f32x4 f[3];
#pragma unroll
    for (int i = 0; i < 3; ++i) f[i] = *reinterpret_cast<const f32x4*>(a.feats + (size_t)row * 768 + (i * 64 + lane) * 4);
    float sh = 0.f, sc = 0.f;
#pragma unroll
    for (int i = 0; i < 3; ++i) {
        const f32x4 w0 = *reinterpret_cast<const f32x4*>(a.shift_w + (i * 64 + lane) * 4);
        const f32x4 w1 = *reinterpret_cast<const f32x4*>(a.scale_w + (i * 64 + lane) * 4);
#pragma unroll
        for (int e = 0; e < 4; ++e) { sh += f[i][e] * w0[e]; sc += f[i][e] * w1[e]; }
    }
    sh = wsum(sh) + a.shift_b[0];
    sc = wsum(sc) + a.scale_b[0];
    sc = (sc > 0.f ? sc : expm1f(sc)) + 1.0f;

    f32x4 c[2];
#pragma unroll
    for (int i = 0; i < 2; ++i) c[i] = *reinterpret_cast<const f32x4*>(a.cls + (size_t)row * 512 + (i * 64 + lane) * 4);
    float n2 = 0.f;
#pragma unroll
    for (int i = 0; i < 2; ++i)
#pragma unroll
        for (int e = 0; e < 4; ++e) n2 += c[i][e] * c[i][e];
    const float den = sqrtf(wsum(n2)) + 1e-6f;
#pragma unroll
    for (int i = 0; i < 2; ++i)
#pragma unroll
        for (int e = 0; e < 4; ++e) c[i][e] = c[i][e] / den;

    const int set = a.image_set ? a.image_set[row / a.np] : 0;
    const int nq = a.setQ[set];
    const float* qn = a.qn + (size_t)set * 32 * 512;
    const uint8_t* qmask = a.qmask + set * 32;
    float best = -FLT_MAX;
    int label = 0;
    for (int q = 0; q < nq; ++q) {
        float d = 0.f;
#pragma unroll
        for (int i = 0; i < 2; ++i) {
            const f32x4 qv = *reinterpret_cast<const f32x4*>(qn + (size_t)q * 512 + (i * 64 + lane) * 4);
#pragma unroll
            for (int e = 0; e < 4; ++e) d += c[i][e] * qv[e];
        }
        d = wsum(d);
        float lg = (d + sh) * sc;
        if (qmask[q] == 0) lg = -FLT_MAX;
        if (a.logits && lane == 0) a.logits[(size_t)row * a.Q + q] = lg;
        if (lg > best) { best = lg; label = q; }
    }

    f32x4 hb[3];
#pragma unroll
    for (int i = 0; i < 3; ++i) hb[i] = *reinterpret_cast<const f32x4*>(a.boxh + (size_t)row * 768 + (i * 64 + lane) * 4);
    float bx[4];
#pragma unroll
    for (int k = 0; k < 4; ++k) {
        float d = 0.f;
#pragma unroll
        for (int i = 0; i < 3; ++i) {
            const f32x4 w = *reinterpret_cast<const f32x4*>(a.box2_w + (size_t)k * 768 + (i * 64 + lane) * 4);
#pragma unroll
            for (int e = 0; e < 4; ++e) d += hb[i][e] * w[e];
        }
        d = wsum(d) + a.box2_b[k] + a.box_bias[p * 4 + k];
        bx[k] = 1.0f / (1.0f + expf(-d));
    }

    if (lane == 0) {
        const float score = 1.0f / (1.0f + expf(-best));
        const float fw = a.box_sx, fh = a.box_sy;
        const float x0 = (bx[0] - 0.5f * bx[2]) * fw, y0 = (bx[1] - 0.5f * bx[3]) * fh;
        const float x1 = (bx[0] + 0.5f * bx[2]) * fw, y1 = (bx[1] + 0.5f * bx[3]) * fh;
        a.scores[row] = score;
        a.labels[row] = label;
        f32x4 o; o[0] = x0; o[1] = y0; o[2] = x1; o[3] = y1;
        *reinterpret_cast<f32x4*>(a.xyxy + (size_t)row * 4) = o;
        if (a.cxcywh) {
            f32x4 bb; bb[0] = bx[0]; bb[1] = bx[1]; bb[2] = bx[2]; bb[3] = bx[3];
            *reinterpret_cast<f32x4*>(a.cxcywh + (size_t)row * 4) = bb;
        }
    }
}

int detect_rows(const DetectRowsArgs& a, hipStream_t s) {
    TSTAR_REQUIRE(a.rows > 0 && a.setQ, "detect_rows: empty problem");
    hipLaunchKernelGGL(detect_rows_kernel, dim3(cdiv(a.rows, 4)), dim3(256), 0, s, a);
    TSTAR_HIP_CHECK(hipGetLastError());
    return TSTAR_OK;
}

__global__ __launch_bounds__(256) void row_dot768_kernel(const float* __restrict__ h, const float* __restrict__ w, const float* __restrict__ b,
                                                         float* __restrict__ out, int rows) {
    const int lane = threadIdx.x & 63;
    const int row = blockIdx.x * 4 + (threadIdx.x >> 6);
    if (row >= rows) return;
    float d = 0.f;
#pragma unroll
    for (int i = 0; i < 3; ++i) {
        const f32x4 x = *reinterpret_cast<const f32x4*>(h + (size_t)row * 768 + (i * 64 + lane) * 4);
        const f32x4 v = *reinterpret_cast<const f32x4*>(w + (i * 64 + lane) * 4);
#pragma unroll
        for (int e = 0; e < 4; ++e) d += x[e] * v[e];
    }
    d = wsum(d) + b[0];
    if (lane == 0) out[row] = d;
}

int row_dot768(const float* h, const float* w, const float* b, float* out, int rows, hipStream_t s) {
    TSTAR_REQUIRE(rows > 0 && h && w && b && out, "row_dot768: empty problem");
    hipLaunchKernelGGL(row_dot768_kernel, dim3(cdiv(rows, 4)), dim3(256), 0, s, h, w, b, out, rows);
    TSTAR_HIP_CHECK(hipGetLastError());
    return TSTAR_OK;
}

__global__ __launch_bounds__(256) void cell_reduce_kernel(const float* __restrict__ scores, const int* __restrict__ labels,
                                                          const float* __restrict__ xyxy, const double* __restrict__ qweight_all,
                                                          const int* __restrict__ image_set, int np, int img_w, int img_h, int grows, int gcols, float thr,
                                                          double* __restrict__ cell_conf, uint32_t* __restrict__ cell_mask,
                                                          int* __restrict__ n_kept) {
    extern __shared__ unsigned long long sm[];
    const int ncell = grows * gcols;
    unsigned long long* cbits = sm;
    uint32_t* cmask = reinterpret_cast<uint32_t*>(sm + ncell);
    __shared__ int kept;
    const int b = blockIdx.x;
    const double* qweight = qweight_all + (image_set ? image_set[b] : 0) * 32;
    for (int i = threadIdx.x; i < ncell; i += blockDim.x) { cbits[i] = 0ull; cmask[i] = 0u; }
    if (threadIdx.x == 0) kept = 0;
    __syncthreads();
    const double cw = (double)img_w / (double)gcols, ch = (double)img_h / (double)grows;
    for (int p = threadIdx.x; p < np; p += blockDim.x) {
        const size_t r = (size_t)b * np + p;
        const float s = scores[r];
        if (s > thr) {
            const int lab = labels[r];
            const double conf = (double)s * qweight[lab];
            const f32x4 bb = *reinterpret_cast<const f32x4*>(xyxy + r * 4);
            const float cx = (bb[0] + bb[2]) * 0.5f;
            const float cy = (bb[1] + bb[3]) * 0.5f;
            int gx = (int)np_floor_divide((double)cx, cw), gy = (int)np_floor_divide((double)cy, ch);
            gx = gx < gcols - 1 ? gx : gcols - 1;
            gy = gy < grows - 1 ? gy : grows - 1;
            gx = gx < 0 ? 0 : gx; gy = gy < 0 ? 0 : gy;
            const int cell = gy * gcols + gx;
            atomicMax(&cbits[cell], (unsigned long long)__double_as_longlong(conf));
            atomicOr(&cmask[cell], 1u << lab);
            atomicAdd(&kept, 1);
        }
    }
    __syncthreads();
    for (int i = threadIdx.x; i < ncell; i += blockDim.x) {
        cell_conf[(size_t)b * ncell + i] = __longlong_as_double((long long)cbits[i]);
        cell_mask[(size_t)b * ncell + i] = cmask[i];
    }
    if (threadIdx.x == 0 && n_kept) n_kept[b] = kept;
}

int cell_reduce(const float* scores, const int* labels, const float* xyxy, const double* qweight, const int* image_set,
                int B, int np, int img_w, int img_h, int grows, int gcols, float thr, double* cell_conf, uint32_t* cell_mask,
                int* n_kept, hipStream_t s) {
    TSTAR_REQUIRE(grows > 0 && gcols > 0 && grows * gcols <= 4096, "cell_reduce: grid must have 1..4096 cells");
    const size_t lds = (size_t)grows * gcols * (sizeof(unsigned long long) + sizeof(uint32_t));
    hipLaunchKernelGGL(cell_reduce_kernel, dim3(B), dim3(256), lds, s, scores, labels, xyxy, qweight, image_set, np, img_w, img_h,
                       grows, gcols, thr, cell_conf, cell_mask, n_kept);
    TSTAR_HIP_CHECK(hipGetLastError());
    return TSTAR_OK;
}

__global__ __launch_bounds__(64) void draw_boxes_kernel(uint8_t* __restrict__ images, int H, int W, const float* __restrict__ xyxy,
                                                        const float* __restrict__ scores, int np, float thr) {
    const int p = blockIdx.x, b = blockIdx.y;
    if (!(scores[(size_t)b * np + p] > thr)) return;
    const f32x4 bb = *reinterpret_cast<const f32x4*>(xyxy + ((size_t)b * np + p) * 4);
    auto pix = [](float v, int hi) { const double r = rint((double)v); return (int)(r < 0.0 ? 0.0 : (r > (double)hi ? (double)hi : r)); };
    const int xa = pix(bb[0], W - 1), ya = pix(bb[1], H - 1), xb = pix(bb[2], W - 1), yb = pix(bb[3], H - 1);
    if (xb < xa || yb < ya) return;
    uint8_t* img = images + (size_t)b * H * W * 3;
    auto put = [&](int x, int y) { uint8_t* q = img + ((size_t)y * W + x) * 3; q[0] = 255; q[1] = 64; q[2] = 64; };
    for (int x = xa + (int)threadIdx.x; x <= xb; x += 64) { put(x, ya); put(x, yb); }
    for (int y = ya + (int)threadIdx.x; y <= yb; y += 64) { put(xa, y); put(xb, y); }
}

int draw_boxes(uint8_t* images, int B, int H, int W, const float* xyxy, const float* scores, int np, float thr, hipStream_t s) {
    TSTAR_REQUIRE(B > 0 && H > 0 && W > 0 && np > 0, "draw_boxes: empty problem");
    hipLaunchKernelGGL(draw_boxes_kernel, dim3(np, B), dim3(64), 0, s, images, H, W, xyxy, scores, np, thr);
    TSTAR_HIP_CHECK(hipGetLastError());
    return TSTAR_OK;
}

}
```

tstar_amd/csrc/kernels.h:

```cpp
#pragma once
#include "common.h"

namespace tstar {

enum { ACT_NONE = 0, ACT_QGELU = 1, ACT_GELU = 2 };

struct GemmArgs {
    const float* A;
    const float* W;
    const __bf16* Wb;
    const void* Wp;
    const void* Wq;
    float* C;
    const float* bias;
    const float* res;
    const float* pos;
    int M, N, K, lda, ldc;
    int act;
    int patch_np;
    int tile_cfg;
    int m_split;
    int group_m;
    int a_terms;
};
int gemm_f32(const GemmArgs& g, hipStream_t stream);

enum GemmTileCfg {
    TILE_AUTO = -1,
    TILE_128 = 0,
    TILE_64N = 1,
    TILE_64 = 2,
    TILE_HYBRID = 3,
    TILE_WIDE = 4,
    TILE_NO_WIDE = 5,
    TILE_WIDE_VW = 6,
    TILE_HYBRID_N = 16,
};

enum GemmWeightMode {
    GEMM_W_F32 = 0,
    GEMM_W_BF16_EXACT = 1,
    GEMM_W_BF16_2T = 3,
    GEMM_W_F32X3 = 4,
};

enum GemmKind {
    GEMM_GRID_128 = 0,
    GEMM_GRID_64N = 1,
    GEMM_GRID_64 = 2,
    GEMM_HYBRID = 3,
    GEMM_WIDE = 4,
    GEMM_WIDE_VW = 5,
};

struct GemmPlan {
    int kind;
    int m_split;
    int blocks;
    int lds_bytes;
    const char* error;
};

GemmPlan plan_gemm(int wmode, int M, int N, int ldc, int patch_np, int tile_cfg, bool has_wq);

int convert_f32_to_bf16(const float* W, __bf16* Wb, __bf16* Wlo, size_t n, hipStream_t s);

int pack_weights_w2(const __bf16* Wb, void* Wq, int N, int K, hipStream_t s);

int pack_weights_x3(const float* W, void* Wp, int N, int K, hipStream_t s);

int layernorm_f32(const float* x, float* y, const float* w, const float* b, int rows, int D, hipStream_t s);

int write_cls_rows(float* x, const float* cls, const float* pos, int B, int ntok, int D, hipStream_t s);

int merge_cls_ln(const float* x, float* feats, const float* post_w, const float* post_b,
                 const float* det_w, const float* det_b, int B, int ntok, int D, hipStream_t s);

int attention_f32(const float* qkv, float* out, int B, int T, int heads, int mode,
                  const uint8_t* key_mask, hipStream_t s);

int attention_split(const float* qkv, float* out, int B, int T, int heads, hipStream_t s);

int attention_x3(const float* qkv, float* out, int B, int T, int heads, hipStream_t s);

}
```

tstar_amd/interface_heuristic.py:

```python
from __future__ import annotations

import os
from dataclasses import dataclass
from typing import Dict, List, Optional

import numpy as np

from . import weights as W
from . import _lib
from .tokenizer import encode_queries


@dataclass
class Detections:
    xyxy: np.ndarray
    confidence: np.ndarray
    class_id: np.ndarray

    def __len__(self) -> int:
        return int(self.xyxy.shape[0])


def _env_int(name: str, default):
    v = os.environ.get(name)
    if v is None or v.strip() == "":
        return default
    try:
        return int(v)
    except ValueError:
        raise ValueError(f"{name} must be an integer, not {v!r}") from None


class HeuristicInterface:
    def __init__(self, heuristic_type: str = "owl-vit", **kwargs):
        """Base of the detector plug-ins (empty in the reference too, interface_heuristic.py:28-37)."""


class OWLInterface(HeuristicInterface):
    def __init__(self, model_name_or_path: str = "google/owlvit-base-patch32", device: str = "cuda",
                 max_batch: Optional[int] = None, synthetic_seed: Optional[int] = None, state_dict: Optional[Dict] = None,
                 weights_dtype: Optional[str] = None, allow_standin_tokenizer: Optional[bool] = None,
                 patch_size: Optional[int] = None, input_size=None, family: Optional[str] = None):
        import torch
        from .owl import OwlScorer
        if not str(device).startswith("cuda"):
            raise ValueError("tstar_amd.OWLInterface runs on the GPU only (device='cuda[:i]'); it has no CPU path")
        if weights_dtype is None:
            weights_dtype = os.environ.get("TSTAR_WEIGHTS_DTYPE") or "f32"
        if weights_dtype not in ("f32", "bf16", "bf16_exact", "f32x3"):
            raise ValueError(f"weights_dtype (or TSTAR_WEIGHTS_DTYPE) must be 'f32', 'bf16', 'bf16_exact' or 'f32x3', not {weights_dtype!r}")
        if max_batch is None:
            max_batch = _env_int("TSTAR_MAX_BATCH", 32)
        if synthetic_seed is None and state_dict is None:
            synthetic_seed = _env_int("TSTAR_SYNTHETIC_SEED", None)
        dev = torch.device(device)
        if dev.index is not None:
            torch.cuda.set_device(dev.index)
        if family is None:
            family = os.environ.get("TSTAR_OWL_FAMILY") or None
        family_given = family is not None
        if family is None:
            family = "owlv2" if "owlv2" in str(model_name_or_path).lower() else "owlvit"
        if family not in W.FAMILIES:
            raise ValueError(f"family (or TSTAR_OWL_FAMILY) must be one of {W.FAMILIES}, not {family!r}")
        if patch_size is not None and not (family == "owlv2" and family_given):
            W.geometry_for_patch(int(patch_size))
        input_size = W.resolve_input_size(input_size)
        if state_dict is None:
            ckpt = W.find_pretrained(model_name_or_path)
            if ckpt is not None:
                geometry = W.geometry_of_checkpoint(ckpt)
                W.with_input_size(geometry, input_size)
                state_dict = W.load_safetensors_state_dict(ckpt)
                self.weights_source = ckpt
            elif synthetic_seed is not None:
                geometry = W.geometry_for_family(family, None if patch_size is None else int(patch_size))
                W.with_input_size(geometry, input_size)
                state_dict = W.synthetic_state_dict(int(synthetic_seed), geometry=geometry)
                self.weights_source = f"synthetic(seed={int(synthetic_seed)})"
            else:
                raise FileNotFoundError(
                    f"no local checkpoint for {model_name_or_path!r} (offline); pass synthetic_seed=<int> "
                    "for seeded synthetic OWL-ViT weights (B/32, or B/16 with patch_size=16; OWLv2 B/16 with family='owlv2' or a "
                    "model name containing 'owlv2') or state_dict=<HF state dict>")
        else:
            geometry = W.geometry_of_state_dict(state_dict)
            self.weights_source = "state_dict"
        if patch_size is not None and int(patch_size) != geometry.patch_size:
            raise ValueError(f"patch_size={int(patch_size)} disagrees with the weights of {self.weights_source!r}, which are "
                             f"{geometry.name} (patch {geometry.patch_size})")
        if family_given and family != geometry.family:
            raise ValueError(f"family={family!r} disagrees with the weights of {self.weights_source!r}, which are {geometry.name} "
                             f"({geometry.family})")
        geometry = W.with_input_size(geometry, input_size)
        self.geometry = geometry
        self.family = geometry.family
        if allow_standin_tokenizer is None:
            allow_standin_tokenizer = self.weights_source.startswith("synthetic(")
        self.allow_standin_tokenizer = bool(allow_standin_tokenizer)
        if weights_dtype in ("bf16", "bf16_exact"):
            state_dict = W.round_weights_to_bf16(state_dict)
        self.weights_dtype = weights_dtype
        self.model_name_or_path = model_name_or_path
# ... 7 lines not shown
        self._ids = None
        self._query_images: Dict[str, np.ndarray] = {}
        self.query_image_info: Dict[str, Dict] = {}

    def set_query_images(self, images: Dict[str, object]):
        import torch
        from PIL import Image
        arrays = {}
        for name, img in images.items():
            key = str(name).strip()
            if not key:
                raise ValueError("set_query_images: an object name must not be blank")
            if isinstance(img, (str, os.PathLike)):
                with Image.open(img) as im:
                    img = np.asarray(im.convert("RGB"), dtype=np.uint8)
            img = np.ascontiguousarray(img)
            if img.dtype != np.uint8 or img.ndim != 3 or img.shape[2] != 3:
                raise ValueError(f"set_query_images: {key!r} must be an HxWx3 uint8 RGB image or a path")
            arrays[key] = img
        by_shape: Dict[tuple, List[str]] = {}
        for key, img in arrays.items():
            by_shape.setdefault(img.shape, []).append(key)
        embeds, info = {}, {}
        for keys in by_shape.values():
            r = self.scorer.embed_image_queries(torch.from_numpy(np.stack([arrays[k] for k in keys])).cuda())
            for i, key in enumerate(keys):
                if int(r.status[i]) == 2:
                    raise ValueError(f"set_query_images: no query can be formed from the example image of {key!r}: none of its "
                                     "predicted boxes overlaps the whole image (empty selection in HF's embed_image_query)")
                embeds[key] = r.embeds[i].copy()
                info[key] = dict(best_index=int(r.best[i]), box_cxcywh=r.boxes_cxcywh[i].copy(), n_selected=int(r.n_selected[i]),
                                 giou_fallback=bool(r.status[i] == 1))
        self._query_images.update(embeds)
        self.query_image_info.update(info)

    def clear_query_images(self):
        self._query_images = {}
        self.query_image_info = {}

    def _image_overrides(self, texts):
        if not self._query_images:
            return None
        return {i: self._query_images[t[0]] for i, t in enumerate(texts[:-1]) if t[0] in self._query_images} or None

    def reparameterize_object_list(self, target_objects: List[str], cue_objects: List[str]):
        combined = list(target_objects) + list(cue_objects)
        self.texts = [[obj.strip()] for obj in combined] + [[' ']]
        ids, am = encode_queries(self.texts, self.model_name_or_path, allow_standin=self.allow_standin_tokenizer)
        self._ids, self._am = ids, am
        w = [1.0] * len(target_objects) + [0.5] * len(cue_objects) + [0.5]
        self.scorer.set_queries(ids, am, w, lazy=True, overrides=self._image_overrides(self.texts))
        self._class_weight = np.asarray(w, dtype=np.float64)

    def inference_detector(self, images, **kwargs) -> List[Detections]:
        import torch
        img = np.array(images[0], dtype=np.uint8, order="C")
        if img.ndim != 3 or img.shape[2] != 3:
            raise ValueError("inference_detector expects HxWx3 uint8 RGB images")
        d_img = torch.from_numpy(img).cuda().unsqueeze(0)
        r = self.scorer.score(d_img, 1, 1)
        dets = [self._detections_from(r, 0)]
        self.detections_inbatch = dets
        return dets

    def inference(self, image_path, use_amp: bool = False) -> Detections:
        from PIL import Image
        with Image.open(image_path) as im:
            image = np.asarray(im.convert("RGB"), dtype=np.uint8)
        return self.inference_detector([image], use_amp=use_amp)[0]

    def bbox_visualization(self, images, detections_inbatch):
        out = []
        for image, det in zip(images, detections_inbatch):
            out.append(draw_boxes(image, det))
        return out

    def set_class_weights(self, object2weight: Dict[str, float]):
        w = [float(object2weight.get(t[0], 0.5)) for t in self.texts]
        self.scorer.set_class_weights(w)
        self._class_weight = np.asarray(w, dtype=np.float64)

    aux_lane = True

    def score_batch(self, d_images, grid_rows: int, grid_cols: int, image_sets=None, lane: int = 0):
        return self.scorer.score(d_images, grid_rows, grid_cols, image_sets=image_sets, lane=lane)

    def install_queries(self, slot: int, target_objects: List[str], cue_objects: List[str],
                        object2weight: Optional[Dict[str, float]] = None) -> List[List[str]]:
        texts, (slot, ids, am, weights, overrides) = self._query_entry(slot, target_objects, cue_objects, object2weight)
        self.scorer.set_queries(ids, am, weights, slot=slot, overrides=overrides)
        return texts

    def _query_entry(self, slot, target_objects, cue_objects, object2weight):
        if not 1 <= int(slot) <= 63:
            raise ValueError("install_queries: slot must be in 1..63")
        texts = [[obj.strip()] for obj in list(target_objects) + list(cue_objects)] + [[' ']]
        ids, am = encode_queries(texts, self.model_name_or_path, allow_standin=self.allow_standin_tokenizer)
        o2w = dict(object2weight or {})
        for o in target_objects:
            o2w.setdefault(o, 1.0)
        for o in cue_objects:
            o2w.setdefault(o, 0.5)
        return texts, (int(slot), ids, am, [float(o2w.get(t[0], 0.5)) for t in texts], self._image_overrides(texts))

    def install_queries_many(self, items) -> List[List[List[str]]]:
        built = [self._query_entry(*it) for it in items]
        self.scorer.set_queries_many([e for _, e in built])
        return [t for t, _ in built]

    def annotated_batch(self, d_images, r, start: int = 0, count: Optional[int] = None):
        count = int(d_images.shape[0]) if count is None else int(count)
        if not d_images.is_contiguous() or d_images.shape[0] != count:
            raise ValueError("annotated_batch: d_images must be a contiguous [count,H,W,3] uint8 device tensor")
        boxes = r.boxes[start:start + count].contiguous()
        scores = r.scores[start:start + count].contiguous()
        lib = _lib.load()
        _lib.check(lib.tstar_draw_boxes_np(d_images.data_ptr(), count, int(d_images.shape[1]), int(d_images.shape[2]),
                                           boxes.data_ptr(), scores.data_ptr(), int(boxes.shape[1]), _lib.stream_ptr()),
                   "tstar_draw_boxes_np")
        imgs = d_images.cpu().numpy()
        s, bx, lab = scores.cpu().numpy(), boxes.cpu().numpy(), r.labels[start:start + count].cpu().numpy()
        dets = []
        for k in range(count):
            keep = s[k] > np.float32(0.005)
            dets.append(Detections(xyxy=bx[k][keep], confidence=s[k][keep], class_id=lab[k][keep].astype(np.int64)))
        return imgs, dets

    def _detections_from(self, r, b: int) -> Detections:
        s = r.scores[b].cpu().numpy()
        keep = s > np.float32(0.005)
        return Detections(xyxy=r.boxes[b].cpu().numpy()[keep], confidence=s[keep],
                          class_id=r.labels[b].cpu().numpy()[keep].astype(np.int64))


def _yolo_scale_from_config(config_path: Optional[str]) -> str:
    import re
    m = re.search(r"yolo_world(?:_v2)?_(s|m|l|xl|x)_", os.path.basename(str(config_path or "")))
    return m.group(1) if m else "l"


class YoloWorldInterface(HeuristicInterface):
    def __init__(self, config_path: Optional[str] = None, checkpoint_path: Optional[str] = None, device: str = "cuda:0", *,
                 scale: Optional[str] = None, synthetic_seed: Optional[int] = None, state_dict: Optional[Dict] = None,
                 text_state_dict: Optional[Dict] = None, max_batch: int = 16):
        import torch
        from .owl import OwlScorer
        from .yolo import YoloDetector
        from . import yolo_world as YW
        if not str(device).startswith("cuda"):
            raise ValueError("tstar_amd.YoloWorldInterface runs on the GPU only (device='cuda[:i]'); it has no CPU path")
        self.config_path, self.checkpoint_path, self.device = config_path, checkpoint_path, device
        self.scale = scale or _yolo_scale_from_config(config_path)
        if state_dict is None and synthetic_seed is None and not (checkpoint_path and os.path.isfile(checkpoint_path)):
            raise FileNotFoundError(
                f"no YOLO-World checkpoint at {checkpoint_path!r} (offline); pass synthetic_seed=<int> for seeded synthetic "
                f"YOLO-World-v2-{self.scale.upper()} weights or state_dict=<mmyolo state dict>")
        dev = torch.device(device)
        if dev.index is not None:
            torch.cuda.set_device(dev.index)
        if state_dict is None and checkpoint_path and os.path.isfile(checkpoint_path):
            ck = torch.load(checkpoint_path, map_location="cpu", weights_only=True)
            ck = ck.get("state_dict", ck)
            state_dict = {k: v.float().numpy() for k, v in ck.items() if hasattr(v, "numpy")}
            self.weights_source = checkpoint_path
        elif state_dict is not None:
            self.weights_source = "state_dict"
        else:
            state_dict = YW.synthetic_state_dict(int(synthetic_seed), self.scale)
            self.weights_source = f"synthetic(seed={int(synthetic_seed)})"
        if text_state_dict is None:
            pre = "backbone.text_model.model."
            clip = {k[len(pre):]: v for k, v in state_dict.items() if k.startswith(pre)}
            if clip:
                text_state_dict = {("owlvit." + k) if not k.startswith("text_projection") else "owlvit." + k: np.asarray(v, np.float32)
                                   for k, v in clip.items()}
                pos = "owlvit.text_model.embeddings.position_embedding.weight"
                if pos in text_state_dict:
                    text_state_dict[pos] = text_state_dict[pos][:W.T_LEN]
            elif self.weights_source.startswith("synthetic("):
                text_state_dict = W.synthetic_state_dict(int(synthetic_seed), "text")
            else:
                raise FileNotFoundError("the YOLO-World state dict carries no CLIP text tower; pass text_state_dict=")
        self.allow_standin_tokenizer = self.weights_source.startswith("synthetic(")
        self.detector = YoloDetector(state_dict, self.scale, max_batch=max_batch)
        self.text_tower = OwlScorer(None, W.pack_blob(text_state_dict, W.text_spec()), max_batch=1)
        self.model_name_or_path = "openai/clip-vit-base-patch32"
        self.texts = []
        self.detections_inbatch: List[Detections] = []
        self._text_feats = None
        self._pending0 = None
        self.set_BBoxAnnotator()

    def set_BBoxAnnotator(self):
        self.BOUNDING_BOX_ANNOTATOR = draw_boxes
        self.LABEL_ANNOTATOR = None

    def _encode(self, texts, weights, slot):
        ids, am = encode_queries(texts, self.model_name_or_path, allow_standin=self.allow_standin_tokenizer)
        self.text_tower.set_queries(ids, am, weights, slot=0)
        feats = self.text_tower.get_query_embeds(0)
        self.detector.set_text_feats(feats, weights, slot=slot)
        return feats

    def reparameterize_object_list(self, target_objects: List[str], cue_objects: List[str]):
        combined = list(target_objects) + list(cue_objects)
        self.texts = [[obj.strip()] for obj in combined] + [[' ']]
        w = [1.0] * len(target_objects) + [0.5] * len(cue_objects) + [0.5]
        ids, am = encode_queries(self.texts, self.model_name_or_path, allow_standin=self.allow_standin_tokenizer)
        self._pending0 = (ids, am, list(w))
        self._text_feats = None
        self._class_weight = np.asarray(w, dtype=np.float64)
# ... 127 lines not shown
```

tstar_amd/interface_searcher.py:

```python
from __future__ import annotations

import os

import ctypes as C
from typing import List, Optional, Tuple

import numpy as np

from . import _lib
from .spline_worker import spline_distribution
from .video import FrameStore, open_video

CELL_W, CELL_H = 200, 95
VERIFY_W, VERIFY_H = 200 * 3, 95 * 3
SAMPLER_WARNING = "Warning: Not enough non-zero entries, adjusting probability distribution."


class _DeviceState:

    def __init__(self, n_frames: int, init_score: float, init_p: float):
        self.lib = _lib.load()
        self.N = n_frames
        h = C.c_void_p()
        _lib.check(self.lib.tstar_searcher_create(C.byref(h), n_frames, init_score, init_p), "tstar_searcher_create")
        self.h = h
        self._vx = np.empty(n_frames + 16, dtype=np.int32)
        self._vy = np.empty(n_frames + 16, dtype=np.float64)

    def close(self):
        if getattr(self, "h", None):
            self.lib.tstar_searcher_destroy(self.h)
            self.h = None

    def __del__(self):
        try:
            self.close()
        except Exception:
            pass

    def apply_grid(self, secs, d_conf) -> Tuple[np.ndarray, np.ndarray]:
        s = np.ascontiguousarray(secs, dtype=np.int32)
        nv = C.c_int(0)
        _lib.check(self.lib.tstar_searcher_apply_grid(self.h, s.ctypes.data, d_conf.data_ptr(), len(s), C.byref(nv),
                                                      self._vx.ctypes.data, self._vy.ctypes.data, _lib.stream_ptr()),
                   "tstar_searcher_apply_grid")
        return self._vx[:nv.value].copy(), self._vy[:nv.value].copy()

    def set_spline(self, t, c, k):
        t = np.ascontiguousarray(t, dtype=np.float64)
        c = np.ascontiguousarray(c, dtype=np.float64)
        if len(c) < len(t):
            c = np.concatenate([c, np.zeros(len(t) - len(c))])
        _lib.check(self.lib.tstar_searcher_set_spline(self.h, t.ctypes.data, c.ctypes.data, len(t), int(k),
                                                      _lib.stream_ptr()), "tstar_searcher_set_spline")

    def sampler_prep(self, num: int, add: float) -> bool:
        fb = C.c_int(0)
        _lib.check(self.lib.tstar_searcher_sampler_prep(self.h, num, add, C.byref(fb), _lib.stream_ptr()),
                   "tstar_searcher_sampler_prep")
        return bool(fb.value)

    def pop_prep(self) -> Tuple[int, float]:
        nnz, tot = C.c_int(0), C.c_double(0.0)
        _lib.check(self.lib.tstar_searcher_pop_prep(self.h, C.byref(nnz), C.byref(tot), _lib.stream_ptr()),
                   "tstar_searcher_pop_prep")
        return int(nnz.value), float(tot.value)

    def window_spread(self, secs, confs, window: int):
        s = np.ascontiguousarray(secs, dtype=np.int32)
        c = np.ascontiguousarray(confs, dtype=np.float64)
        if s.shape != c.shape or s.ndim != 1:
            raise ValueError("window_spread: one confidence per sampled frame")
        if len(s) == 0:
            return
        _lib.check(self.lib.tstar_searcher_window_spread(self.h, s.ctypes.data, c.ctypes.data, len(s), int(window),
                                                         _lib.stream_ptr()), "tstar_searcher_window_spread")

    def visited(self) -> Tuple[np.ndarray, np.ndarray]:
        nv = C.c_int(0)
        _lib.check(self.lib.tstar_searcher_visited(self.h, C.byref(nv), self._vx.ctypes.data, self._vy.ctypes.data,
                                                   _lib.stream_ptr()), "tstar_searcher_visited")
        return self._vx[:nv.value].copy(), self._vy[:nv.value].copy()

    def write(self, which: int, values):
        v = np.ascontiguousarray(values, dtype=np.float64)
        if v.shape != (self.N,):
            raise ValueError(f"searcher state arrays have length {self.N}")
        _lib.check(self.lib.tstar_searcher_write(self.h, int(which), v.ctypes.data, _lib.stream_ptr()), "tstar_searcher_write")

    def draw(self, x) -> np.ndarray:
        x = np.ascontiguousarray(x, dtype=np.float64)
        out = np.empty(len(x), dtype=np.int32)
        _lib.check(self.lib.tstar_searcher_draw(self.h, x.ctypes.data, len(x), out.ctypes.data, _lib.stream_ptr()),
                   "tstar_searcher_draw")
        return out

    def exclude(self, found):
# ... 276 lines not shown
                        break

    def _update_from_device(self, secs: List[int], d_conf, overlap=None):
        vx, vy = self._state.apply_grid(secs, d_conf)
        if overlap is not None:
            from . import spline_pool
            wait = spline_pool.distribution_async([(vx, vy)], [self.total_frame_num])
            try:
                ctx = overlap()
            except BaseException:
                wait()
                raise
            P = wait()[0]
        else:
            ctx = None
            P = spline_distribution(vx, vy, self.total_frame_num)
        self._state.write(2, P)
        self.store_score_distribution()
        return ctx

    def update_top_25_with_window(self, frame_confidences, sampled_frame_indices, window_size: int = 5):
        self._state.window_spread([int(i) for i in sampled_frame_indices], [float(c) for c in frame_confidences],
                                  window_size)

    def spline_keyframe_distribution(self, non_visiting_frames, score_distribution, video_length: int) -> np.ndarray:
        non_visiting_frames = np.asarray(non_visiting_frames)
        visited = np.nonzero(non_visiting_frames == 0)[0]
        return spline_distribution(visited, np.asarray(score_distribution, dtype=np.float64)[visited], int(video_length))

    def update_frame_distribution(self, sampled_frame_indices, confidence_maps, detected_objects_maps):
        import torch
        confidence_map = np.asarray(confidence_maps[0], dtype=np.float64)
        detected_objects_map = detected_objects_maps[0]
        _, grid_cols = self.image_grid_shape
        secs = [int(s) for s in sampled_frame_indices]
        frame_confidences = [confidence_map[i // grid_cols, i % grid_cols] for i in range(len(secs))]
        frame_detected_objects = [detected_objects_map[i] for i in range(len(secs))]
        d_conf = torch.tensor(frame_confidences, dtype=torch.float64, device=self.store.frames.device)
        self._update_from_device(secs, d_conf)
        return frame_confidences, frame_detected_objects

    def sample_frames(self, num_samples: int):
        secs = self._sample_secs(num_samples)
        return secs, _ResizedFrames(self, secs, CELL_W * 4, CELL_H * 4)

    def _sample_secs(self, num_samples: int, _warned: Optional[list] = None) -> List[int]:
        pre = getattr(self, "_prefetched_secs", None)
        if pre is not None:
            self._prefetched_secs = None
            secs, post_state, warned = pre
            (self._rng if self._rng is not None else np.random).set_state(post_state)
            if warned:
                print(SAMPLER_WARNING)
            return secs
        if num_samples > self.total_frame_num:
            num_samples = self.total_frame_num
        if not self.Score_history:
            interval = self.total_frame_num // num_samples
            secs = np.arange(0, self.total_frame_num, interval)[:num_samples]
            if len(secs) < num_samples:
                secs = np.append(secs, self.total_frame_num - 1)
        else:
            if self._state.sampler_prep(num_samples, num_samples / self.total_frame_num):
                if _warned is not None:
                    _warned.append(True)
                else:
                    print(SAMPLER_WARNING)
            secs = self._choice(num_samples)
        return [int(s) for s in secs]

    def pop_frames(self, video_path, num_samples: int):
        nnz, total = self._state.pop_prep()
        secs = self._choice(num_samples, nnz, total)
        secs.sort()
        time_stamps = [sec / self.fps for sec in secs]
        frames = self.store.host_frames(secs)
        return frames, time_stamps

    def _verify_launch(self, secs: List[int], names_per_frame: List[List[str]]):
        cands = [i for i, names in enumerate(names_per_frame) if any(t in names for t in self.remaining_targets)]
        if not cands:
            return None
        vframes = self._device_verify_frames([secs[i] for i in cands])
        res = self.heuristic.score_batch(vframes, 1, 1)
        self.device_images_scored += len(cands)
        return cands, vframes, res

    def _verify_finish(self, ctx, secs: List[int], names_per_frame: List[List[str]]):
        if ctx is None:
            return
        cands, vframes, res = ctx
        vconf = res.cell_conf[:, 0].cpu().numpy()
        vmask = res.cell_mask[:, 0].cpu().numpy().astype(np.uint32)
        self._verify_replay(cands, vconf, vmask, secs, names_per_frame, vframes, res, 0)

    def _verify_replay(self, cands, vconf, vmask, secs, names_per_frame, vframes=None, res=None, res_offset=0):
        slot = {i: j for j, i in enumerate(cands)}
        upd_s, upd_v = [], []
        hist = None
        for i, (sec, names) in enumerate(zip(secs, names_per_frame)):
            for target in list(self.remaining_targets):
                if target in names:
                    j = slot[i]
                    single_conf = vconf[j]
                    single_names = self._names_from_mask(int(vmask[j]))
                    upd_s.append(sec)
                    upd_v.append(single_conf)
                    self.frames_scored += 1
                    self.detector_calls += 1
                    if self.keep_visual_history and res is not None:
                        if hist is None:
                            hist = self.heuristic.annotated_batch(vframes[res_offset:res_offset + len(cands)], res,
                                                                  res_offset, len(cands))
                        frame, det = hist[0][j], hist[1][j]
                        self.image_grid_iters.append([frame])
                        self.detect_annotot_iters.append([frame])
                        self.detect_bbox_iters.append([det])
                    if target in single_names and single_conf > self.confidence_threshold:
                        self.remaining_targets.remove(target)
                        print(f"Found target '{target}' in frame {int(sec * self.raw_fps / self.fps)}, score {single_conf:.2f}")
                        break
        if upd_s:
            self._state.set_scores(upd_s, upd_v)

    def verify_and_remove_target(self, frame_sec: int, detected_objects: List[str], confidence_threshold: float) -> bool:
        for target in list(self.remaining_targets):
            if target in detected_objects:
                d_frame = self._device_verify_frames([int(frame_sec)])
                if self._fast:
                    res = self.heuristic.score_batch(d_frame, 1, 1)
                    single_conf = float(res.cell_conf[0, 0].item())
                    single_names = self._names_from_mask(int(res.cell_mask[0, 0].item()) & 0xFFFFFFFF)
                    det = self.heuristic._detections_from(res, 0) if self.keep_visual_history else None
                else:
                    conf_map, det_map = self.score_image_grids([d_frame[0].cpu().numpy()], (1, 1))
                    single_conf, single_names = conf_map[0, 0, 0], det_map[0][0]
                    det = None
                self._state.set_scores([int(frame_sec)], [single_conf])
                self.frames_scored += 1
                self.detector_calls += 1
                self.device_images_scored += 1
                if self.keep_visual_history:
                    frame = d_frame[0].cpu().numpy()
                    dets = [det] if det is not None else self.heuristic.detections_inbatch
                    self.image_grid_iters.append([frame])
                    self.detect_annotot_iters.append(self.heuristic.bbox_visualization([frame], dets))
                    self.detect_bbox_iters.append(dets)
                if target in single_names and single_conf > confidence_threshold:
                    self.remaining_targets.remove(target)
                    print(f"Found target '{target}' in frame {int(frame_sec * self.raw_fps / self.fps)}, score {single_conf:.2f}")
                    return True
        return False

    def _verify_generic(self, secs, names_per_frame):
        for sec, names in zip(secs, names_per_frame):
            for target in list(self.remaining_targets):
                if target in names:
                    frame = self._device_verify_frames([sec])[0].cpu().numpy()
                    conf_map, det_map = self.score_image_grids([frame], (1, 1))
                    single_conf = conf_map[0, 0, 0]
                    self._state.set_scores([sec], [single_conf])
                    self.frames_scored += 1
                    self.detector_calls += 1
                    self.device_images_scored += 1
                    if self.keep_visual_history:
                        self.image_grid_iters.append([frame])
                        self.detect_annotot_iters.append(self.heuristic.bbox_visualization(
                            images=[frame], detections_inbatch=self.heuristic.detections_inbatch))
                        self.detect_bbox_iters.append(self.heuristic.detections_inbatch)
                    if target in det_map[0][0] and single_conf > self.confidence_threshold:
                        self.remaining_targets.remove(target)
                        print(f"Found target '{target}' in frame {int(sec * self.raw_fps / self.fps)}, score {single_conf:.2f}")
                        break

    def search(self):
        import torch
        if self._fast and os.environ.get("TSTAR_SOLO_SEQUENTIAL") is None:
            from .lockstep import search_solo
            return search_solo(self)
        while self.remaining_targets and self.search_budget > 0:
            rows, cols = self.image_grid_shape
            n = rows * cols
            secs, _lazy_frames = self.sample_frames(n)
            secs = [int(s_) for s_ in secs]
            self.search_budget -= n
            grid = self._device_grid(secs)
            if self._fast:
                res = self.heuristic.score_batch(grid.unsqueeze(0), rows, cols)
                self.device_images_scored += 1
                d_conf = res.cell_conf[0]
                masks = res.cell_mask[0].cpu().numpy().astype(np.uint32)
                names_per_frame = [self._names_from_mask(int(m)) for m in masks[:len(secs)]]
                if self.keep_visual_history:
                    imgs, dets = self.heuristic.annotated_batch(grid.unsqueeze(0), res, 0, 1)
                    self.heuristic.detections_inbatch = dets
                    self.image_grid_iters.append([imgs[0]])
                    self.detect_annotot_iters.append([imgs[0]])
                    self.detect_bbox_iters.append(dets)
            else:
                g = grid.cpu().numpy()
                conf_maps, name_maps = self.score_image_grids([g], self.image_grid_shape)
                self.device_images_scored += 1
                d_conf = torch.from_numpy(np.ascontiguousarray(conf_maps[0].reshape(-1))).to(grid.device)
                names_per_frame = [name_maps[0][i] for i in range(len(secs))]
                if self.keep_visual_history:
                    self.image_grid_iters.append([g])
                    self.detect_annotot_iters.append(self.heuristic.bbox_visualization(
                        images=[g], detections_inbatch=self.heuristic.detections_inbatch))
                    self.detect_bbox_iters.append(self.heuristic.detections_inbatch)
            self.frames_scored += n
            self.detector_calls += 1
            if self._fast:
                ctx = self._update_from_device(secs, d_conf, lambda: self._verify_launch(secs, names_per_frame))
# ... 29 lines not shown
```

tstar_amd/lockstep.py:

```python
from __future__ import annotations

import os
from typing import List, Sequence, Tuple

import numpy as np

from . import spline_pool
from .interface_searcher import CELL_H, CELL_W, SAMPLER_WARNING, VERIFY_H, VERIFY_W, TStarSearcher

MAX_GROUP = 63

_SIDE = {}
_AUX = {}
_SPECULATE = os.environ.get("TSTAR_NO_SPECULATION") is None
_BESIDE = os.environ.get("TSTAR_SPECULATE_BEHIND") is None
_AHEAD = os.environ.get("TSTAR_NO_VERIFY_AHEAD") is None
_AHEAD_ALWAYS = False
_ONE_UPLOAD = os.environ.get("TSTAR_PER_ITEM_UPLOADS") is None
AUX_IMAGES = 31
_GROUP_BESIDE = os.environ.get("TSTAR_GROUP_GRIDS_BESIDE") is not None


def _side_stream(torch):
    d = torch.cuda.current_device()
    if d not in _SIDE:
        _SIDE[d] = torch.cuda.Stream(device=d)
    return _SIDE[d]


def _accepts_lane(fn) -> bool:
    import inspect
    try:
        ps = inspect.signature(fn).parameters
    except (TypeError, ValueError):
        return False
    return "lane" in ps or any(p.kind == inspect.Parameter.VAR_KEYWORD for p in ps.values())


def _aux_stream(torch):
    d = torch.cuda.current_device()
    if d not in _AUX:
        _AUX[d] = torch.cuda.Stream(device=d)
    return _AUX[d]


class _Group:

    def __init__(self, searchers: Sequence[TStarSearcher], first_slot: int, torch):
        self.torch = torch
        self.ss = list(searchers)
        self.h = self.ss[0].heuristic
        self.rows, self.cols = tuple(self.ss[0].image_grid_shape)
        self.n = self.rows * self.cols
        for i, s in enumerate(self.ss):
            s._slot = first_slot + i
        self.main = torch.cuda.current_stream()
        self.side = _side_stream(torch)
        self.aux = _aux_stream(torch) if (_BESIDE and getattr(self.h, "aux_lane", False) and _accepts_lane(self.h.score_batch)) else None
        self.pending = None
        self.act = []
        self.spec = None
        self.spec_beside = False
        self.grids_beside = False
        self.ahead = None
        self.vq = self.masks = None
        self.solo = False

    def install(self):
        h = self.h
        self.side.wait_stream(self.main)
        if self.aux is not None:
            self.aux.wait_stream(self.main)
        if self.solo:
            self.act = self._active()
            return
        if hasattr(h, "install_queries_many"):
            texts = h.install_queries_many([(s._slot, s.target_objects, s.cue_objects, s.object2weight) for s in self.ss])
            for s, t in zip(self.ss, texts):
                s._texts = t
        else:
            for s in self.ss:
                s._texts = h.install_queries(s._slot, s.target_objects, s.cue_objects, s.object2weight)
        self.act = self._active()

    def _active(self):
        return [s for s in self.ss if s.remaining_targets and s.search_budget > 0]

    def _sets(self, items):
        return None if self.solo else [s._slot for s in items]

    def _draw(self, s):
# ... 55 lines not shown
            self.ev_grid.record(stream)

    def _grid_batch(self, items, secs_l):
        torch = self.torch
        if not _ONE_UPLOAD:
            grids = [s._device_grid(secs) for s, secs in zip(items, secs_l)]
            return torch.stack(grids), grids
        dev = items[0].store.frames.device
        n = self.n
        for secs in secs_l:
            if len(secs) != n:
                raise ValueError("Frame count does not match grid dimensions")
        d_idx = torch.as_tensor([int(v) for secs in secs_l for v in secs], dtype=torch.int32, device=dev)
        batch = torch.empty((len(items), self.rows * CELL_H, self.cols * CELL_W, 3), dtype=torch.uint8, device=dev)
        for i, s in enumerate(items):
            s._device_grid_into(d_idx[i * n:(i + 1) * n], batch[i])
        return batch, [batch[i] for i in range(len(items))]

    def speculate(self):
        torch = self.torch
        items = [s for s in self.act if s.remaining_targets and s.search_budget > 0]
        if not items or len(items) != len(self.act):
            return
        states = [(s._rng if s._rng is not None else np.random).get_state() for s in items]
        secs_l, grids, warned = [], [], []
        with torch.cuda.stream(self.side):
            for s in items:
                w = []
                secs_l.append(s._sample_secs(self.n, _warned=w))
                warned.append(bool(w and w[0]))
                s.search_budget -= self.n
        beside = self.aux is not None and len(items) <= AUX_IMAGES
        stream = self.aux if beside else self.main
        with torch.cuda.stream(stream):
            batch, grids = self._grid_batch(items, secs_l)
            if beside:
                res = self.h.score_batch(batch, self.rows, self.cols, image_sets=self._sets(items), lane=1)
            else:
                res = self.h.score_batch(batch, self.rows, self.cols, image_sets=self._sets(items))
            ev = torch.cuda.Event()
            ev.record(stream)
        self.spec = (items, secs_l, grids, res, ev, states, warned)
        self.spec_beside = beside

    def _drop_speculation(self):
        if self.ahead is not None:
            self._drop_ahead()
        items, _, _, res, _, states, _ = self.spec
        self.spec = None
        for s, st in zip(items, states):
            (s._rng if s._rng is not None else np.random).set_state(st)
            s.search_budget += self.n
            s.device_images_scored += 1
        cb = getattr(self.h, "_speculation_dropped", None)
        if cb is not None:
            cb(res)

    def _verify_queue(self, act, secs_l, res, ev_grid):
        torch, h = self.torch, self.h
        with torch.cuda.stream(self.side):
            self.side.wait_event(ev_grid)
            masks = res.cell_mask.cpu().numpy().astype(np.uint32)
        cand_l = []
        for i, s in enumerate(act):
            tb = 0
            for q, t in enumerate(s._texts):
                if t[0] in s.remaining_targets:
                    tb |= 1 << q
            cand_l.append(np.nonzero(masks[i][:len(secs_l[i])] & np.uint32(tb))[0].tolist())
        vres = vframes = ev = None
        offs = np.cumsum([0] + [len(c) for c in cand_l])
        if offs[-1] > 0:
            if _ONE_UPLOAD:
                dev = act[0].store.frames.device
                d_idx = torch.as_tensor([secs_l[i][j] for i in range(len(act)) for j in cand_l[i]], dtype=torch.int32, device=dev)
                vframes = torch.empty((int(offs[-1]), VERIFY_H, VERIFY_W, 3), dtype=torch.uint8, device=dev)
                for i, s in enumerate(act):
                    if cand_l[i]:
                        s._device_resized_into(d_idx[int(offs[i]):int(offs[i + 1])], vframes[int(offs[i]):int(offs[i + 1])])
            else:
                vframes = torch.cat([s._device_verify_frames([secs_l[i][j] for j in cand_l[i]])
                                     for i, s in enumerate(act) if cand_l[i]])
            sets = None if self.solo else [s._slot for i, s in enumerate(act) for _ in cand_l[i]]
            vres = h.score_batch(vframes, 1, 1, image_sets=sets)
            ev = torch.cuda.Event()
            ev.record(self.main)
        return masks, (vres, vframes, ev, cand_l, offs, [list(s.remaining_targets) for s in act])

    def middle(self):
        self.verify_launch()
        self.update()

    def verify_launch(self):
        if self.ahead is not None:
            self.masks, self.vq = self.ahead
            self.ahead = None
            return
        self.masks, self.vq = self._verify_queue(self.act, self.secs_l, self.res, self.ev_grid)

    def verify_ahead(self):
        if self.spec is None or self.ahead is not None:
            return
        items, secs_l, _, res, ev, _, _ = self.spec
        self.ahead = self._verify_queue(items, secs_l, res, ev)

    def verification_done(self) -> bool:
        ev = self.vq[2] if self.vq is not None else None
        return ev is None or ev.query()

    def _drop_ahead(self):
        _, (vres, _, _, cand_l, _, _) = self.ahead
        self.ahead = None
        for s, c in zip(self.spec[0] if self.spec is not None else self.act, cand_l):
            s.device_images_scored += len(c)
        cb = getattr(self.h, "_speculation_dropped", None)
        if cb is not None and vres is not None:
            cb(vres)

    def update(self):
        torch, h, act, res, secs_l, n, masks = self.torch, self.h, self.act, self.res, self.secs_l, self.n, self.masks
        names_l, fits = [], []
        with torch.cuda.stream(self.side):
            for i, s in enumerate(act):
                names_l.append([s._names_from_mask(int(m)) for m in masks[i][:len(secs_l[i])]])
                s.device_images_scored += 1
                if s.keep_visual_history:
                    imgs, dets = h.annotated_batch(self.grids[i].unsqueeze(0), res, i, 1)
                    if self.solo:
                        h.detections_inbatch = dets
                    s.image_grid_iters.append([imgs[0]])
                    s.detect_annotot_iters.append([imgs[0]])
                    s.detect_bbox_iters.append(dets)
                s.frames_scored += n
                s.detector_calls += 1
                fits.append(s._state.apply_grid(secs_l[i], res.cell_conf[i]))
        with torch.cuda.stream(self.side):
            for s, P in zip(act, spline_pool.distribution_many(fits, [a.total_frame_num for a in act], s=0.5)):
                s._state.write(2, P)
            for s in act:
                if type(s).store_score_distribution is TStarSearcher.store_score_distribution:
                    s.store_score_distribution(_defer_lists=True)
                else:
                    s.store_score_distribution()
        vres, vframes, ev, cand_l, offs, _ = self.vq
        self.pending = (vres, vframes, ev, cand_l, offs, names_l)

    def end(self):
        for s in self.act:
            s._finalize_history()
        if self.pending is None:
            if self.spec is not None:
                self._drop_speculation()
            return
        torch = self.torch
        vres, vframes, ev, cand_l, offs, names_l = self.pending
        self.pending = None
        act, secs_l = self.act, self.secs_l
        if vres is not None:
            with torch.cuda.stream(self.side):
                self.side.wait_event(ev)
                vconf = vres.cell_conf[:, 0].cpu().numpy()
                vmask = vres.cell_mask[:, 0].cpu().numpy().astype(np.uint32)
                for i, s in enumerate(act):
                    if cand_l[i]:
                        s.device_images_scored += len(cand_l[i])
                        s._verify_replay(cand_l[i], vconf[offs[i]:offs[i + 1]], vmask[offs[i]:offs[i + 1]], secs_l[i],
                                         names_l[i], vframes, vres, int(offs[i]))
# ... 96 lines not shown
```

tstar_amd/owl.py:

```python
from __future__ import annotations

import ctypes as C
from dataclasses import dataclass
from typing import Optional, Sequence

import numpy as np

from . import _lib
from . import weights as W

OPENAI_CLIP_MEAN = (0.48145466, 0.4578275, 0.40821073)
OPENAI_CLIP_STD = (0.26862954, 0.26130258, 0.27577711)


FAMILY_CODES = {"owlvit": 0, "owlv2": 1}


def owlv2_axis_radius(S: int, out: int) -> int:
    sigma = max(0.0, (S / out - 1) / 2)
    return -1 if sigma <= 1e-15 else int(4.0 * sigma + 0.5)


def owlv2_gaussian_half(S: int, out: int) -> np.ndarray:
    lw = owlv2_axis_radius(S, out)
# ... 163 lines not shown
        if not entries:
            return
        overrides = [self._check_overrides(e[4] if len(e) > 4 else None, np.shape(e[1])[0]) for e in entries]
        slots = np.ascontiguousarray([int(e[0]) for e in entries], dtype=np.int32)
        ids = [np.ascontiguousarray(e[1], dtype=np.int32) for e in entries]
        am = [np.ascontiguousarray(e[2], dtype=np.int32) for e in entries]
        w = [np.ascontiguousarray(e[3], dtype=np.float64) for e in entries]
        for i_, a_, w_ in zip(ids, am, w):
            if i_.ndim != 2 or i_.shape[1] != W.T_LEN or a_.shape != i_.shape or w_.shape != (i_.shape[0],):
                raise ValueError("set_queries_many: ids/mask must be [Q,16] and class_weight [Q] per entry")
        Qs = np.ascontiguousarray([i_.shape[0] for i_ in ids], dtype=np.int32)
        ids_c, am_c, w_c = np.concatenate(ids), np.concatenate(am), np.concatenate(w)
        rc = self._lib.tstar_owl_set_queries_many(self._h, len(entries), slots.ctypes.data, Qs.ctypes.data, ids_c.ctypes.data, am_c.ctypes.data,
                                                  w_c.ctypes.data, _lib.stream_ptr())
        _lib.check(rc, "tstar_owl_set_queries_many")
        for sl, q in zip(slots, Qs):
            self._pending.pop(int(sl), None)
            self.Qs[int(sl)] = int(q)
        for sl, i_, w_, ov in zip(slots, ids, w, overrides):
            self._apply_overrides(int(sl), i_, w_, ov)

    def set_query_embeds(self, embeds: np.ndarray, query_mask: Sequence[int], class_weight: Sequence[float], slot: int = 0):
        e = np.ascontiguousarray(embeds, dtype=np.float32)
        m = np.ascontiguousarray(query_mask, dtype=np.uint8)
        w = np.ascontiguousarray(class_weight, dtype=np.float64)
        Q = e.shape[0]
        if e.shape != (Q, W.PROJ) or m.shape != (Q,) or w.shape != (Q,):
            raise ValueError("set_query_embeds: embeds [Q,512], mask [Q], class_weight [Q]")
        self._pending.pop(int(slot), None)
        rc = self._lib.tstar_owl_set_query_embeds(self._h, int(slot), e.ctypes.data, m.ctypes.data, w.ctypes.data, Q,
                                                  _lib.stream_ptr())
        _lib.check(rc, "tstar_owl_set_query_embeds")
        self.Qs[int(slot)] = Q

    def set_class_weights(self, class_weight: Sequence[float], slot: int = 0):
        w = np.ascontiguousarray(class_weight, dtype=np.float64)
        if w.shape != (self.Qs.get(int(slot), 0),):
            raise ValueError("set_class_weights: one weight per installed query")
        if int(slot) in self._pending:
            p = self._pending[int(slot)]
            self._pending[int(slot)] = (p[0], p[1], w.copy(), p[3])
            return
        rc = self._lib.tstar_owl_set_class_weights(self._h, int(slot), w.ctypes.data, len(w), _lib.stream_ptr())
        _lib.check(rc, "tstar_owl_set_class_weights")

    def get_query_embeds(self, slot: int = 0) -> np.ndarray:
        self._flush([slot])
        q = self.Qs.get(int(slot), 0)
        out = np.empty((q, W.PROJ), dtype=np.float32)
        rc = self._lib.tstar_owl_get_query_embeds(self._h, int(slot), out.ctypes.data, q, _lib.stream_ptr())
        _lib.check(rc, "tstar_owl_get_query_embeds")
        return out

    def embed_image_queries(self, images) -> ImageQueryResult:
        torch = self._torch
        if images.dtype != torch.uint8 or images.dim() != 4 or images.shape[-1] != 3 or not images.is_cuda:
            raise ValueError("embed_image_queries: images must be a cuda uint8 tensor [n,H,W,3]")
        images = images.contiguous()
        n, H, Wd, _ = images.shape
        if n < 1:
            raise ValueError("embed_image_queries: no image")
        r = ImageQueryResult(embeds=np.zeros((n, W.PROJ), np.float32), best=np.zeros(n, np.int32), boxes_cxcywh=np.zeros((n, 4), np.float32),
                             n_selected=np.zeros(n, np.int32), status=np.zeros(n, np.int32))
        if self.family == "owlv2":
            self._prepare_v2(H, Wd)
        rc = self._lib.tstar_owl_embed_image_queries(self._h, images.data_ptr(), n, H, Wd, r.embeds.ctypes.data, r.best.ctypes.data,
                                                     r.boxes_cxcywh.ctypes.data, r.n_selected.ctypes.data, r.status.ctypes.data, _lib.stream_ptr())
        _lib.check(rc, "tstar_owl_embed_image_queries")
        return r

    def _prepare_v2(self, H: int, Wd: int):
        S = max(int(H), int(Wd))
        done = self.__dict__.setdefault("_v2_axes", set())
        for out in (self.geometry.input_h, self.geometry.input_w):
            if (S, out) in done or S < 2:
                continue
            if owlv2_axis_radius(S, out) > 0:
                gw = owlv2_gaussian_half(S, out)
                _lib.check(self._lib.tstar_owlv2_set_axis_weights(self._h, S, out, gw.ctypes.data, int(gw.size)),
                           "tstar_owlv2_set_axis_weights")
            done.add((S, out))

    def score(self, images, grid_rows: int, grid_cols: int, want_logits: bool = False,
              image_sets: Optional[Sequence[int]] = None, lane: int = 0, objectness: bool = False) -> ScoreResult:
        torch = self._torch
        if images.dtype != torch.uint8 or images.dim() != 4 or images.shape[-1] != 3 or not images.is_cuda:
            raise ValueError("score: images must be a cuda uint8 tensor [B,H,W,3]")
        if grid_rows < 1 or grid_cols < 1:
            raise ValueError("score: the grid must be at least 1x1")
        images = images.contiguous()
        B, H, Wd, _ = images.shape
        dev = images.device
        ncell = grid_rows * grid_cols
        npatch = self.num_patches
        r = ScoreResult(
            scores=torch.empty((B, npatch), dtype=torch.float32, device=dev),
            labels=torch.empty((B, npatch), dtype=torch.int32, device=dev),
            boxes=torch.empty((B, npatch, 4), dtype=torch.float32, device=dev),
            cell_conf=torch.empty((B, ncell), dtype=torch.float64, device=dev),
            cell_mask=torch.empty((B, ncell), dtype=torch.int32, device=dev),
            n_kept=torch.empty((B,), dtype=torch.int32, device=dev),
        )
        sets = None
        if image_sets is not None:
            sets = np.ascontiguousarray(image_sets, dtype=np.int32)
            if sets.shape != (B,):
                raise ValueError("score: image_sets needs one slot per image")
        if self._pending:
            self._flush(sets.tolist() if sets is not None else [0])
        if want_logits:
            qs = {self.Qs.get(int(v), 0) for v in (sets if sets is not None else [0])}
            if len(qs) != 1:
                raise ValueError("score: raw logits need the same query count for every image")
            r.logits = torch.empty((B, npatch, qs.pop()), dtype=torch.float32, device=dev)
            r.boxes_cxcywh = torch.empty((B, npatch, 4), dtype=torch.float32, device=dev)
        if objectness:
            if self.family != "owlv2":
                raise ValueError("score: objectness needs an OWLv2 scorer (OWL-ViT has no objectness head)")
            r.objectness = torch.empty((B, npatch), dtype=torch.float32, device=dev)
        if self.family == "owlv2":
            self._prepare_v2(H, Wd)
        rc = self._lib.tstar_owl_score_lane_obj(
            self._h, int(lane), images.data_ptr(), B, H, Wd, grid_rows, grid_cols,
            None if sets is None else sets.ctypes.data, r.scores.data_ptr(), r.labels.data_ptr(), r.boxes.data_ptr(), r.cell_conf.data_ptr(),
            r.cell_mask.data_ptr(), r.n_kept.data_ptr(),
            _lib.ptr(r.logits), _lib.ptr(r.boxes_cxcywh), _lib.ptr(r.objectness), _lib.stream_ptr())
        _lib.check(rc, "tstar_owl_score")
        return r

    def debug_preprocess(self, images):
        torch = self._torch
        images = images.contiguous()
        B, H, Wd, _ = images.shape
        if self.family == "owlv2":
            self._prepare_v2(H, Wd)
            pat = torch.empty((B * self.num_patches, self.geometry.patch_k), dtype=torch.float32, device=images.device)
            rc = self._lib.tstar_owl_debug_preprocess(self._h, images.data_ptr(), B, H, Wd, None, pat.data_ptr(), _lib.stream_ptr())
            _lib.check(rc, "tstar_owl_debug_preprocess")
            return None, pat
        u8 = torch.empty((B, self.geometry.input_h, self.geometry.input_w, 3), dtype=torch.uint8, device=images.device)
        pat = torch.empty((B * self.num_patches, self.geometry.patch_k), dtype=torch.float32, device=images.device)
        rc = self._lib.tstar_owl_debug_preprocess(self._h, images.data_ptr(), B, H, Wd, u8.data_ptr(),
                                                  pat.data_ptr(), _lib.stream_ptr())
        _lib.check(rc, "tstar_owl_debug_preprocess")
        return u8, pat

    def preprocess_form(self, lane: int = 0) -> int:
        return int(self._lib.tstar_owlv2_last_preprocess_form(self._h, int(lane)))
```

Measured before the change: 11940.

## Skip box-head GEMMs for 1x1 verify scoring and add XCD-grouped attention order

```diff
diff --git a/include/tstar_hip.h b/include/tstar_hip.h
--- a/include/tstar_hip.h
+++ b/include/tstar_hip.h
@@ -71,6 +71,10 @@
                              const int32_t* h_image_query_set, float* d_scores, int32_t* d_labels, float* d_boxes_xyxy,
                              double* d_cell_conf, uint32_t* d_cell_mask, int32_t* d_n_kept, float* d_logits,
                              float* d_boxes_cxcywh, float* d_objectness, void* stream);
+
+int tstar_owl_score_cells(tstar_owl* h, int lane, const uint8_t* d_images, int B, int H, int W, int grid_rows, int grid_cols,
+                          const int32_t* h_image_query_set, float* d_scores, int32_t* d_labels, double* d_cell_conf,
+                          uint32_t* d_cell_mask, int32_t* d_n_kept, float* d_logits, float* d_objectness, void* stream);
 
 int tstar_owlv2_set_axis_weights(tstar_owl* h, int S, int out, const double* gw, int n);
 int tstar_owlv2_preprocess_plan(int H, int W, int out_h, int out_w, int* plan10);
@@ -208,6 +212,9 @@
 
 int tstar_attention_split(const float* d_qkv, float* d_out, int B, int T, int heads, void* stream);
 int tstar_attention_x3(const float* d_qkv, float* d_out, int B, int T, int heads, void* stream);
+int tstar_attention_x3_order(const float* d_qkv, float* d_out, int B, int T, int heads, int order, void* stream);
+int tstar_xcd_group_block(int bid, int ngroups, int gsize);
+int tstar_xcd_groups_grid(int ngroups, int gsize);
 
 int tstar_prof_enable(int on);
 int tstar_prof_read(int category, long long* launches, double* total_ms, double* total_flops);
diff --git a/tstar_amd/_lib.py b/tstar_amd/_lib.py
--- a/tstar_amd/_lib.py
+++ b/tstar_amd/_lib.py
@@ -26,6 +26,7 @@
     "tstar_owl_create_family": (_i, [C.POINTER(_vp), _i, _i, _i, _i, _vp, _sz, _vp, _sz, _vp, _i, _i]),
     "tstar_owl_vision_blob_floats_family": (_sz, [_i, _i, _i, _i]),
     "tstar_owl_score_lane_obj": (_i, [_vp, _i, _vp, _i, _i, _i, _i, _i, _vp, _vp, _vp, _vp, _vp, _vp, _vp, _vp, _vp, _vp, _vp]),
+    "tstar_owl_score_cells": (_i, [_vp, _i, _vp, _i, _i, _i, _i, _i, _vp, _vp, _vp, _vp, _vp, _vp, _vp, _vp, _vp]),
     "tstar_owlv2_set_axis_weights": (_i, [_vp, _i, _i, _vp, _i]),
     "tstar_owlv2_preprocess_plan": (_i, [_i, _i, _i, _i, C.POINTER(_i)]),
     "tstar_owlv2_axis_window": (_i, [_i, _i, _i, _i, _i, C.POINTER(_i)]),
@@ -106,6 +107,9 @@
     "tstar_draw_boxes_np": (_i, [_vp, _i, _i, _i, _vp, _vp, _i, _vp]),
     "tstar_attention_split": (_i, [_vp, _vp, _i, _i, _i, _vp]),
     "tstar_attention_x3": (_i, [_vp, _vp, _i, _i, _i, _vp]),
+    "tstar_attention_x3_order": (_i, [_vp, _vp, _i, _i, _i, _i, _vp]),
+    "tstar_xcd_group_block": (_i, [_i, _i, _i]),
+    "tstar_xcd_groups_grid": (_i, [_i, _i]),
     "tstar_attention_f32": (_i, [_vp, _vp, _i, _i, _i, _i, _vp, _vp]),
     "tstar_prof_enable": (_i, [_i]),
     "tstar_prof_read": (_i, [_i, _vp, _vp, _vp]),
diff --git a/tstar_amd/csrc/attention_x3.h b/tstar_amd/csrc/attention_x3.h
--- a/tstar_amd/csrc/attention_x3.h
+++ b/tstar_amd/csrc/attention_x3.h
@@ -2,6 +2,7 @@
 #include <hip/hip_runtime.h>
 #include <math.h>
 #include <utility>
+#include "common.h"
 
 namespace tstar {
 namespace ax3 {
@@ -53,13 +54,14 @@
 
 template <bool PLANES>
 __global__ __launch_bounds__(256, 2) void attention_x3_kernel(const float* __restrict__ qkv, const char* __restrict__ planes,
-                                                              float* __restrict__ out, int T, int heads, int qtiles) {
+                                                              float* __restrict__ out, int T, int heads, int qtiles, int xcd_groups) {
     extern __shared__ __attribute__((aligned(16))) char smem[];
     char* const kbuf = smem;
     char* const vbuf = smem + NKB * KBUF;
 
     const int D = heads * HD, D3 = 3 * D;
-    int bid = blockIdx.x;
+    int bid = xcd_groups ? xcd_remap_groups(blockIdx.x, xcd_groups, qtiles) : (int)blockIdx.x;
+    if (bid < 0) return;
     const int qt = bid % qtiles; bid /= qtiles;
     const int head = bid % heads;
     const int b = bid / heads;
@@ -476,8 +478,11 @@
 }
 #endif
 
-inline int attention_x3_launch(const float* qkv, float* out, int B, int T, int heads, hipStream_t s, const char* planes = nullptr) {
+inline int attention_x3_launch(const float* qkv, float* out, int B, int T, int heads, hipStream_t s, const char* planes = nullptr,
+                               bool xcd_order = false) {
     const int qtiles = (T + 127) / 128;
+    const int xcd_groups = xcd_order ? B * heads : 0;
+    const int nblocks = xcd_order ? xcd_groups_grid(B * heads, qtiles) : B * heads * qtiles;
 #ifdef TSTAR_ATTN_X3_LAB
     static bool attr[2] = {false, false};
     if (planes) {
@@ -486,7 +491,7 @@
             if (e != hipSuccess) return (int)e;
             attr[1] = true;
         }
-        hipLaunchKernelGGL(ax3::attention_x3_kernel<true>, dim3(B * heads * qtiles), dim3(256), ax3::LDS_BYTES, s, qkv, planes, out, T, heads, qtiles);
+        hipLaunchKernelGGL(ax3::attention_x3_kernel<true>, dim3(nblocks), dim3(256), ax3::LDS_BYTES, s, qkv, planes, out, T, heads, qtiles, xcd_groups);
         return (int)hipGetLastError();
     }
     if (!attr[0]) {
@@ -496,7 +501,7 @@
     }
 #endif
     if (planes) return (int)hipErrorInvalidValue;
-    hipLaunchKernelGGL(ax3::attention_x3_kernel<false>, dim3(B * heads * qtiles), dim3(256), ax3::LDS_BYTES, s, qkv, planes, out, T, heads, qtiles);
+    hipLaunchKernelGGL(ax3::attention_x3_kernel<false>, dim3(nblocks), dim3(256), ax3::LDS_BYTES, s, qkv, planes, out, T, heads, qtiles, xcd_groups);
     return (int)hipGetLastError();
 }
 
diff --git a/tstar_amd/csrc/attention_x3.hip b/tstar_amd/csrc/attention_x3.hip
--- a/tstar_amd/csrc/attention_x3.hip
+++ b/tstar_amd/csrc/attention_x3.hip
@@ -1,3 +1,4 @@
+#include <stdlib.h>
 #include "common.h"
 #include "kernels.h"
 #include "prof.h"
@@ -5,13 +6,15 @@
 
 namespace tstar {
 
-int attention_x3(const float* qkv, float* out, int B, int T, int heads, hipStream_t s) {
+int attention_x3(const float* qkv, float* out, int B, int T, int heads, hipStream_t s, int order) {
     TSTAR_REQUIRE(B > 0 && T > 0 && heads > 0, "attention_x3: empty problem");
     TSTAR_REQUIRE(((size_t)T + 32) * 3 * heads * 64 * 4 < (1ull << 31), "attention_x3: one image's qkv rows (plus one key tile of look-ahead) must stay below 2 GiB");
     if (int rc = ensure_dyn_lds(reinterpret_cast<const void*>(ax3::attention_x3_kernel<false>), ax3::LDS_BYTES)) return rc;
     const bool prof = prof_enabled();
     if (prof) prof_start(PROF_ATTN, s, 4.0 * B * heads * (double)T * T * 64);
-    const int rc = attention_x3_launch(qkv, out, B, T, heads, s);
+    static const bool xcd_off = getenv("TSTAR_AX3_XCD_OFF") != nullptr;
+    const bool xcd_order = order < 0 ? !xcd_off : order != 0;
+    const int rc = attention_x3_launch(qkv, out, B, T, heads, s, nullptr, xcd_order);
     if (prof) prof_stop(PROF_ATTN, s);
     TSTAR_HIP_CHECK((hipError_t)rc);
     return TSTAR_OK;
diff --git a/tstar_amd/csrc/capi.hip b/tstar_amd/csrc/capi.hip
--- a/tstar_amd/csrc/capi.hip
+++ b/tstar_amd/csrc/capi.hip
@@ -336,7 +336,8 @@
     float* bh1;
     float* bh2;
 };
-static int owl_forward_heads(tstar_owl* h, tstar_owl::Lane& L, const uint8_t* d_images, int Bc, int H, int W, OwlHeadTensors* t, hipStream_t s) {
+static int owl_forward_heads(tstar_owl* h, tstar_owl::Lane& L, const uint8_t* d_images, int Bc, int H, int W, bool want_boxes, OwlHeadTensors* t,
+                             hipStream_t s) {
     const OwlGeom& G = h->geom;
     const int NP = G.np, NTOK = G.ntok, PK = G.patch_k;
     const int M = Bc * NTOK, MP = Bc * NP;
@@ -350,6 +351,7 @@
     t->feats = L.xn; t->cls = L.att; t->bh1 = L.qkv; t->bh2 = L.hid;
     RC(merge_cls_ln(L.x, t->feats, h->vw.post_ln_w, h->vw.post_ln_b, h->vw.det_ln_w, h->vw.det_ln_b, Bc, NTOK, V_D, s));
     RC(gemm_f32(mk_gemm(h, t->feats, h->vw.cls_w, t->cls, h->vw.cls_b, nullptr, MP, PROJ, V_D, V_D, PROJ, ACT_NONE), s));
+    if (!want_boxes) return TSTAR_OK;
     RC(gemm_f32(mk_gemm(h, t->feats, h->vw.box0_w, t->bh1, h->vw.box0_b, nullptr, MP, V_D, V_D, V_D, V_D, ACT_GELU), s));
     RC(gemm_f32(mk_gemm(h, t->bh1, h->vw.box1_w, t->bh2, h->vw.box1_b, nullptr, MP, V_D, V_D, V_D, V_D, ACT_GELU), s));
     return TSTAR_OK;
@@ -725,25 +727,10 @@
     return TSTAR_OK;
 }
 
-int tstar_owl_score(tstar_owl* h, const uint8_t* d_images, int B, int H, int W, int grid_rows, int grid_cols,
-                    const int32_t* h_image_query_set, float* d_scores, int32_t* d_labels, float* d_boxes_xyxy, double* d_cell_conf,
-                    uint32_t* d_cell_mask, int32_t* d_n_kept, float* d_logits, float* d_boxes_cxcywh, void* stream) {
-    return tstar_owl_score_lane(h, 0, d_images, B, H, W, grid_rows, grid_cols, h_image_query_set, d_scores, d_labels, d_boxes_xyxy, d_cell_conf,
-                                d_cell_mask, d_n_kept, d_logits, d_boxes_cxcywh, stream);
-}
-
-int tstar_owl_score_lane(tstar_owl* h, int lane, const uint8_t* d_images, int B, int H, int W, int grid_rows, int grid_cols,
-                         const int32_t* h_image_query_set, float* d_scores, int32_t* d_labels, float* d_boxes_xyxy, double* d_cell_conf,
-                         uint32_t* d_cell_mask, int32_t* d_n_kept, float* d_logits, float* d_boxes_cxcywh, void* stream) {
-    return tstar_owl_score_lane_obj(h, lane, d_images, B, H, W, grid_rows, grid_cols, h_image_query_set, d_scores, d_labels, d_boxes_xyxy, d_cell_conf,
-                                    d_cell_mask, d_n_kept, d_logits, d_boxes_cxcywh, nullptr, stream);
-}
-
-int tstar_owl_score_lane_obj(tstar_owl* h, int lane, const uint8_t* d_images, int B, int H, int W, int grid_rows, int grid_cols,
-                             const int32_t* h_image_query_set, float* d_scores, int32_t* d_labels, float* d_boxes_xyxy, double* d_cell_conf,
-                             uint32_t* d_cell_mask, int32_t* d_n_kept, float* d_logits, float* d_boxes_cxcywh, float* d_objectness, void* stream) {
-    TSTAR_REQUIRE(h && d_images && d_scores && d_labels && d_boxes_xyxy && d_cell_conf && d_cell_mask,
-                  "tstar_owl_score: null argument");
+static int owl_score(tstar_owl* h, int lane, const uint8_t* d_images, int B, int H, int W, int grid_rows, int grid_cols,
+                     const int32_t* h_image_query_set, float* d_scores, int32_t* d_labels, float* d_boxes_xyxy, double* d_cell_conf,
+                     uint32_t* d_cell_mask, int32_t* d_n_kept, float* d_logits, float* d_boxes_cxcywh, float* d_objectness, void* stream) {
+    const bool want_boxes = d_boxes_xyxy != nullptr;
     TSTAR_REQUIRE(lane >= 0 && lane < TSTAR_OWL_LANES, "tstar_owl_score_lane: lane must be 0 or 1");
     TSTAR_REQUIRE(B >= 1 && H >= 1 && W >= 1, "tstar_owl_score: empty batch or image");
     TSTAR_REQUIRE(grid_rows >= 1 && grid_cols >= 1, "tstar_owl_score: grid must be at least 1x1");
@@ -780,13 +767,13 @@
         const int Bc = (B - b0) < L.cap ? (B - b0) : L.cap;
         const int MP = Bc * NP;
         OwlHeadTensors t;
-        RC(owl_forward_heads(h, L, d_images + (size_t)b0 * H * W * 3, Bc, H, W, &t, s));
+        RC(owl_forward_heads(h, L, d_images + (size_t)b0 * H * W * 3, Bc, H, W, want_boxes, &t, s));
         float *feats = t.feats, *cls = t.cls, *bh1 = t.bh1, *bh2 = t.bh2;
         DetectRowsArgs a = detect_args(h);
-        a.feats = feats; a.cls = cls; a.boxh = bh2;
+        a.feats = feats; a.cls = cls; a.boxh = want_boxes ? bh2 : nullptr;
         a.scores = d_scores + (size_t)b0 * NP;
         a.labels = d_labels + (size_t)b0 * NP;
-        a.xyxy = d_boxes_xyxy + (size_t)b0 * NP * 4;
+        a.xyxy = want_boxes ? d_boxes_xyxy + (size_t)b0 * NP * 4 : nullptr;
         a.logits = d_logits ? d_logits + (size_t)b0 * NP * q_uniform : nullptr;
         a.image_set = h_image_query_set ? L.d_image_set + b0 : nullptr;
         a.cxcywh = d_boxes_cxcywh ? d_boxes_cxcywh + (size_t)b0 * NP * 4 : nullptr;
@@ -805,6 +792,39 @@
     return TSTAR_OK;
 }
 
+int tstar_owl_score(tstar_owl* h, const uint8_t* d_images, int B, int H, int W, int grid_rows, int grid_cols,
+                    const int32_t* h_image_query_set, float* d_scores, int32_t* d_labels, float* d_boxes_xyxy, double* d_cell_conf,
+                    uint32_t* d_cell_mask, int32_t* d_n_kept, float* d_logits, float* d_boxes_cxcywh, void* stream) {
+    return tstar_owl_score_lane(h, 0, d_images, B, H, W, grid_rows, grid_cols, h_image_query_set, d_scores, d_labels, d_boxes_xyxy, d_cell_conf,
+                                d_cell_mask, d_n_kept, d_logits, d_boxes_cxcywh, stream);
+}
+
+int tstar_owl_score_lane(tstar_owl* h, int lane, const uint8_t* d_images, int B, int H, int W, int grid_rows, int grid_cols,
+                         const int32_t* h_image_query_set, float* d_scores, int32_t* d_labels, float* d_boxes_xyxy, double* d_cell_conf,
+                         uint32_t* d_cell_mask, int32_t* d_n_kept, float* d_logits, float* d_boxes_cxcywh, void* stream) {
+    return tstar_owl_score_lane_obj(h, lane, d_images, B, H, W, grid_rows, grid_cols, h_image_query_set, d_scores, d_labels, d_boxes_xyxy, d_cell_conf,
+                                    d_cell_mask, d_n_kept, d_logits, d_boxes_cxcywh, nullptr, stream);
+}
+
+int tstar_owl_score_lane_obj(tstar_owl* h, int lane, const uint8_t* d_images, int B, int H, int W, int grid_rows, int grid_cols,
+                             const int32_t* h_image_query_set, float* d_scores, int32_t* d_labels, float* d_boxes_xyxy, double* d_cell_conf,
+                             uint32_t* d_cell_mask, int32_t* d_n_kept, float* d_logits, float* d_boxes_cxcywh, float* d_objectness, void* stream) {
+    TSTAR_REQUIRE(h && d_images && d_scores && d_labels && d_boxes_xyxy && d_cell_conf && d_cell_mask,
+                  "tstar_owl_score: null argument");
+    return owl_score(h, lane, d_images, B, H, W, grid_rows, grid_cols, h_image_query_set, d_scores, d_labels, d_boxes_xyxy, d_cell_conf, d_cell_mask,
+                     d_n_kept, d_logits, d_boxes_cxcywh, d_objectness, stream);
+}
+
+int tstar_owl_score_cells(tstar_owl* h, int lane, const uint8_t* d_images, int B, int H, int W, int grid_rows, int grid_cols,
+                          const int32_t* h_image_query_set, float* d_scores, int32_t* d_labels, double* d_cell_conf, uint32_t* d_cell_mask,
+                          int32_t* d_n_kept, float* d_logits, float* d_objectness, void* stream) {
+    TSTAR_REQUIRE(h && d_images && d_scores && d_labels && d_cell_conf && d_cell_mask, "tstar_owl_score_cells: null argument");
+    TSTAR_REQUIRE(grid_rows >= 1 && grid_cols >= 1, "tstar_owl_score: grid must be at least 1x1");
+    TSTAR_REQUIRE(grid_rows * grid_cols == 1, "tstar_owl_score_cells: only a 1x1 grid can be scored without boxes (the cell of a detection is its box centre's)");
+    return owl_score(h, lane, d_images, B, H, W, grid_rows, grid_cols, h_image_query_set, d_scores, d_labels, nullptr, d_cell_conf, d_cell_mask,
+                     d_n_kept, d_logits, nullptr, d_objectness, stream);
+}
+
 int tstar_owl_debug_preprocess(tstar_owl* h, const uint8_t* d_images, int B, int H, int W, uint8_t* d_out_u8,
                                float* d_out_patches, void* stream) {
     TSTAR_REQUIRE(h && d_images && d_out_patches, "tstar_owl_debug_preprocess: null argument");
@@ -946,7 +966,7 @@
         const int Bc = (n - b0) < L.cap ? (n - b0) : L.cap;
         const int MP = Bc * NP;
         OwlHeadTensors t;
-        rc = owl_forward_heads(h, L, d_images + (size_t)b0 * H * W * 3, Bc, H, W, &t, s);
+        rc = owl_forward_heads(h, L, d_images + (size_t)b0 * H * W * 3, Bc, H, W, true, &t, s);
         if (rc) break;
         const size_t R = round_up((size_t)MP, 4);
         DetectRowsArgs a = detect_args(h);
@@ -1234,6 +1254,18 @@
     return attention_x3(d_qkv, d_out, B, T, heads, (hipStream_t)stream);
 }
 
+int tstar_attention_x3_order(const float* d_qkv, float* d_out, int B, int T, int heads, int order, void* stream) {
+    TSTAR_REQUIRE(d_qkv && d_out, "tstar_attention_x3_order: null argument");
+    TSTAR_REQUIRE(order == 0 || order == 1, "tstar_attention_x3_order: order must be 0 (linear) or 1 (XCD groups)");
+    return attention_x3(d_qkv, d_out, B, T, heads, (hipStream_t)stream, order);
+}
+
+int tstar_xcd_group_block(int bid, int ngroups, int gsize) {
+    if (bid < 0 || ngroups < 1 || gsize < 1 || bid >= xcd_groups_grid(ngroups, gsize)) return -2;
+    return xcd_remap_groups(bid, ngroups, gsize);
+}
+int tstar_xcd_groups_grid(int ngroups, int gsize) { return ngroups < 1 || gsize < 1 ? -1 : xcd_groups_grid(ngroups, gsize); }
+
 int tstar_attention_split(const float* d_qkv, float* d_out, int B, int T, int heads, void* stream) {
     TSTAR_REQUIRE(d_qkv && d_out, "tstar_attention_split: null argument");
     return attention_split(d_qkv, d_out, B, T, heads, (hipStream_t)stream);
diff --git a/tstar_amd/csrc/common.h b/tstar_amd/csrc/common.h
--- a/tstar_amd/csrc/common.h
+++ b/tstar_amd/csrc/common.h
@@ -33,12 +33,19 @@
 typedef float f32x4 __attribute__((ext_vector_type(4)));
 typedef float f32x16 __attribute__((ext_vector_type(16)));
 
-__device__ __forceinline__ int xcd_remap(int bid, int nwg) {
+__host__ __device__ __forceinline__ int xcd_remap(int bid, int nwg) {
     const int nx = 8;
     int xcd = bid % nx, idx = bid / nx;
     int q = nwg / nx, r = nwg % nx;
     int base = (xcd < r) ? xcd * (q + 1) : r * (q + 1) + (xcd - r) * q;
     return base + idx;
+}
+
+static inline int xcd_groups_grid(int ngroups, int gsize) { return (ngroups + 7) / 8 * 8 * gsize; }
+__host__ __device__ __forceinline__ int xcd_remap_groups(int bid, int ngroups, int gsize) {
+    const int xcd = bid % 8, idx = bid / 8;
+    const int slot = (idx / gsize) * 8 + xcd;
+    return slot < ngroups ? xcd_remap(slot, ngroups) * gsize + idx % gsize : -1;
 }
 
 __device__ __forceinline__ void store_px4(uint8_t* d, const unsigned (&v)[4][3]) {
diff --git a/tstar_amd/csrc/heads.hip b/tstar_amd/csrc/heads.hip
--- a/tstar_amd/csrc/heads.hip
+++ b/tstar_amd/csrc/heads.hip
@@ -67,41 +67,47 @@
         if (lg > best) { best = lg; label = q; }
     }
 
-    f32x4 hb[3];
-#pragma unroll
-    for (int i = 0; i < 3; ++i) hb[i] = *reinterpret_cast<const f32x4*>(a.boxh + (size_t)row * 768 + (i * 64 + lane) * 4);
-    float bx[4];
-#pragma unroll
-    for (int k = 0; k < 4; ++k) {
-        float d = 0.f;
-#pragma unroll
-        for (int i = 0; i < 3; ++i) {
-            const f32x4 w = *reinterpret_cast<const f32x4*>(a.box2_w + (size_t)k * 768 + (i * 64 + lane) * 4);
-#pragma unroll
-            for (int e = 0; e < 4; ++e) d += hb[i][e] * w[e];
-        }
-        d = wsum(d) + a.box2_b[k] + a.box_bias[p * 4 + k];
-        bx[k] = 1.0f / (1.0f + expf(-d));
+    float bx[4] = {0.f, 0.f, 0.f, 0.f};
+    const bool boxes = a.boxh != nullptr;
+    if (boxes) {
+        f32x4 hb[3];
+#pragma unroll
+        for (int i = 0; i < 3; ++i) hb[i] = *reinterpret_cast<const f32x4*>(a.boxh + (size_t)row * 768 + (i * 64 + lane) * 4);
+#pragma unroll
+        for (int k = 0; k < 4; ++k) {
+            float d = 0.f;
+#pragma unroll
+            for (int i = 0; i < 3; ++i) {
+                const f32x4 w = *reinterpret_cast<const f32x4*>(a.box2_w + (size_t)k * 768 + (i * 64 + lane) * 4);
+#pragma unroll
+                for (int e = 0; e < 4; ++e) d += hb[i][e] * w[e];
+            }
+            d = wsum(d) + a.box2_b[k] + a.box_bias[p * 4 + k];
+            bx[k] = 1.0f / (1.0f + expf(-d));
+        }
     }
 
     if (lane == 0) {
         const float score = 1.0f / (1.0f + expf(-best));
-        const float fw = a.box_sx, fh = a.box_sy;
-        const float x0 = (bx[0] - 0.5f * bx[2]) * fw, y0 = (bx[1] - 0.5f * bx[3]) * fh;
-        const float x1 = (bx[0] + 0.5f * bx[2]) * fw, y1 = (bx[1] + 0.5f * bx[3]) * fh;
         a.scores[row] = score;
         a.labels[row] = label;
-        f32x4 o; o[0] = x0; o[1] = y0; o[2] = x1; o[3] = y1;
-        *reinterpret_cast<f32x4*>(a.xyxy + (size_t)row * 4) = o;
-        if (a.cxcywh) {
-            f32x4 bb; bb[0] = bx[0]; bb[1] = bx[1]; bb[2] = bx[2]; bb[3] = bx[3];
-            *reinterpret_cast<f32x4*>(a.cxcywh + (size_t)row * 4) = bb;
+        if (boxes) {
+            const float fw = a.box_sx, fh = a.box_sy;
+            const float x0 = (bx[0] - 0.5f * bx[2]) * fw, y0 = (bx[1] - 0.5f * bx[3]) * fh;
+            const float x1 = (bx[0] + 0.5f * bx[2]) * fw, y1 = (bx[1] + 0.5f * bx[3]) * fh;
+            f32x4 o; o[0] = x0; o[1] = y0; o[2] = x1; o[3] = y1;
+            *reinterpret_cast<f32x4*>(a.xyxy + (size_t)row * 4) = o;
+            if (a.cxcywh) {
+                f32x4 bb; bb[0] = bx[0]; bb[1] = bx[1]; bb[2] = bx[2]; bb[3] = bx[3];
+                *reinterpret_cast<f32x4*>(a.cxcywh + (size_t)row * 4) = bb;
+            }
         }
     }
 }
 
 int detect_rows(const DetectRowsArgs& a, hipStream_t s) {
     TSTAR_REQUIRE(a.rows > 0 && a.setQ, "detect_rows: empty problem");
+    TSTAR_REQUIRE(a.boxh ? a.xyxy != nullptr : !a.cxcywh, "detect_rows: box outputs go with the box head's hidden rows");
     hipLaunchKernelGGL(detect_rows_kernel, dim3(cdiv(a.rows, 4)), dim3(256), 0, s, a);
     TSTAR_HIP_CHECK(hipGetLastError());
     return TSTAR_OK;
@@ -153,14 +159,17 @@
         if (s > thr) {
             const int lab = labels[r];
             const double conf = (double)s * qweight[lab];
-            const f32x4 bb = *reinterpret_cast<const f32x4*>(xyxy + r * 4);
-            const float cx = (bb[0] + bb[2]) * 0.5f;
-            const float cy = (bb[1] + bb[3]) * 0.5f;
-            int gx = (int)np_floor_divide((double)cx, cw), gy = (int)np_floor_divide((double)cy, ch);
-            gx = gx < gcols - 1 ? gx : gcols - 1;
-            gy = gy < grows - 1 ? gy : grows - 1;
-            gx = gx < 0 ? 0 : gx; gy = gy < 0 ? 0 : gy;
-            const int cell = gy * gcols + gx;
+            int cell = 0;
+            if (xyxy) {
+                const f32x4 bb = *reinterpret_cast<const f32x4*>(xyxy + r * 4);
+                const float cx = (bb[0] + bb[2]) * 0.5f;
+                const float cy = (bb[1] + bb[3]) * 0.5f;
+                int gx = (int)np_floor_divide((double)cx, cw), gy = (int)np_floor_divide((double)cy, ch);
+                gx = gx < gcols - 1 ? gx : gcols - 1;
+                gy = gy < grows - 1 ? gy : grows - 1;
+                gx = gx < 0 ? 0 : gx; gy = gy < 0 ? 0 : gy;
+                cell = gy * gcols + gx;
+            }
             atomicMax(&cbits[cell], (unsigned long long)__double_as_longlong(conf));
             atomicOr(&cmask[cell], 1u << lab);
             atomicAdd(&kept, 1);
@@ -178,6 +187,7 @@
                 int B, int np, int img_w, int img_h, int grows, int gcols, float thr, double* cell_conf, uint32_t* cell_mask,
                 int* n_kept, hipStream_t s) {
     TSTAR_REQUIRE(grows > 0 && gcols > 0 && grows * gcols <= 4096, "cell_reduce: grid must have 1..4096 cells");
+    TSTAR_REQUIRE(xyxy || grows * gcols == 1, "cell_reduce: a grid of more than one cell needs the boxes");
     const size_t lds = (size_t)grows * gcols * (sizeof(unsigned long long) + sizeof(uint32_t));
     hipLaunchKernelGGL(cell_reduce_kernel, dim3(B), dim3(256), lds, s, scores, labels, xyxy, qweight, image_set, np, img_w, img_h,
                        grows, gcols, thr, cell_conf, cell_mask, n_kept);
diff --git a/tstar_amd/csrc/kernels.h b/tstar_amd/csrc/kernels.h
--- a/tstar_amd/csrc/kernels.h
+++ b/tstar_amd/csrc/kernels.h
@@ -81,6 +81,6 @@
 
 int attention_split(const float* qkv, float* out, int B, int T, int heads, hipStream_t s);
 
-int attention_x3(const float* qkv, float* out, int B, int T, int heads, hipStream_t s);
+int attention_x3(const float* qkv, float* out, int B, int T, int heads, hipStream_t s, int order = -1);
 
 }
diff --git a/tstar_amd/interface_heuristic.py b/tstar_amd/interface_heuristic.py
--- a/tstar_amd/interface_heuristic.py
+++ b/tstar_amd/interface_heuristic.py
@@ -19,6 +19,9 @@
 
     def __len__(self) -> int:
         return int(self.xyxy.shape[0])
+
+
+NO_BOXES_ERROR = "this result was scored with boxes=False and holds no boxes; score the images with boxes=True to draw or list detections"
 
 
 def _env_int(name: str, default):
@@ -192,8 +195,8 @@
 
     aux_lane = True
 
-    def score_batch(self, d_images, grid_rows: int, grid_cols: int, image_sets=None, lane: int = 0):
-        return self.scorer.score(d_images, grid_rows, grid_cols, image_sets=image_sets, lane=lane)
+    def score_batch(self, d_images, grid_rows: int, grid_cols: int, image_sets=None, lane: int = 0, boxes: bool = True):
+        return self.scorer.score(d_images, grid_rows, grid_cols, image_sets=image_sets, lane=lane, boxes=boxes)
 
     def install_queries(self, slot: int, target_objects: List[str], cue_objects: List[str],
                         object2weight: Optional[Dict[str, float]] = None) -> List[List[str]]:
@@ -222,6 +225,8 @@
         count = int(d_images.shape[0]) if count is None else int(count)
         if not d_images.is_contiguous() or d_images.shape[0] != count:
             raise ValueError("annotated_batch: d_images must be a contiguous [count,H,W,3] uint8 device tensor")
+        if r.boxes is None:
+            raise ValueError("annotated_batch: " + NO_BOXES_ERROR)
         boxes = r.boxes[start:start + count].contiguous()
         scores = r.scores[start:start + count].contiguous()
         lib = _lib.load()
@@ -237,6 +242,8 @@
         return imgs, dets
 
     def _detections_from(self, r, b: int) -> Detections:
+        if r.boxes is None:
+            raise ValueError("_detections_from: " + NO_BOXES_ERROR)
         s = r.scores[b].cpu().numpy()
         keep = s > np.float32(0.005)
         return Detections(xyxy=r.boxes[b].cpu().numpy()[keep], confidence=s[keep],
diff --git a/tstar_amd/interface_searcher.py b/tstar_amd/interface_searcher.py
--- a/tstar_amd/interface_searcher.py
+++ b/tstar_amd/interface_searcher.py
@@ -13,6 +13,29 @@
 
 CELL_W, CELL_H = 200, 95
 VERIFY_W, VERIFY_H = 200 * 3, 95 * 3
+_ACCEPTS = {}
+
+
+def accepts_keyword(fn, name: str) -> bool:
+    import inspect
+    key = (getattr(fn, "__func__", fn), name)
+    if key not in _ACCEPTS:
+        try:
+            ps = inspect.signature(fn).parameters
+            _ACCEPTS[key] = name in ps or any(p.kind == inspect.Parameter.VAR_KEYWORD for p in ps.values())
+        except (TypeError, ValueError):
+            _ACCEPTS[key] = False
+    return _ACCEPTS[key]
+
+
+def verify_score_kwargs(heuristic, keep_boxes: bool) -> dict:
+    fn = heuristic.score_batch
+    own = getattr(fn, "__self__", None) is heuristic and "score_batch" not in vars(heuristic)
+    if keep_boxes or not own or not accepts_keyword(fn, "boxes"):
+        return {}
+    return {"boxes": False}
+
+
 SAMPLER_WARNING = "Warning: Not enough non-zero entries, adjusting probability distribution."
 
 
@@ -455,7 +478,7 @@
         if not cands:
             return None
         vframes = self._device_verify_frames([secs[i] for i in cands])
-        res = self.heuristic.score_batch(vframes, 1, 1)
+        res = self.heuristic.score_batch(vframes, 1, 1, **verify_score_kwargs(self.heuristic, self.keep_visual_history))
         self.device_images_scored += len(cands)
         return cands, vframes, res
 
@@ -501,7 +524,7 @@
             if target in detected_objects:
                 d_frame = self._device_verify_frames([int(frame_sec)])
                 if self._fast:
-                    res = self.heuristic.score_batch(d_frame, 1, 1)
+                    res = self.heuristic.score_batch(d_frame, 1, 1, **verify_score_kwargs(self.heuristic, self.keep_visual_history))
                     single_conf = float(res.cell_conf[0, 0].item())
                     single_names = self._names_from_mask(int(res.cell_mask[0, 0].item()) & 0xFFFFFFFF)
                     det = self.heuristic._detections_from(res, 0) if self.keep_visual_history else None
diff --git a/tstar_amd/lockstep.py b/tstar_amd/lockstep.py
--- a/tstar_amd/lockstep.py
+++ b/tstar_amd/lockstep.py
@@ -6,7 +6,7 @@
 import numpy as np
 
 from . import spline_pool
-from .interface_searcher import CELL_H, CELL_W, SAMPLER_WARNING, VERIFY_H, VERIFY_W, TStarSearcher
+from .interface_searcher import CELL_H, CELL_W, SAMPLER_WARNING, VERIFY_H, VERIFY_W, TStarSearcher, verify_score_kwargs
 
 MAX_GROUP = 63
 
@@ -228,7 +228,7 @@
                 vframes = torch.cat([s._device_verify_frames([secs_l[i][j] for j in cand_l[i]])
                                      for i, s in enumerate(act) if cand_l[i]])
             sets = None if self.solo else [s._slot for i, s in enumerate(act) for _ in cand_l[i]]
-            vres = h.score_batch(vframes, 1, 1, image_sets=sets)
+            vres = h.score_batch(vframes, 1, 1, image_sets=sets, **verify_score_kwargs(h, any(s.keep_visual_history for s in act)))
             ev = torch.cuda.Event()
             ev.record(self.main)
         return masks, (vres, vframes, ev, cand_l, offs, [list(s.remaining_targets) for s in act])
diff --git a/tstar_amd/owl.py b/tstar_amd/owl.py
--- a/tstar_amd/owl.py
+++ b/tstar_amd/owl.py
@@ -269,12 +269,14 @@
             done.add((S, out))
 
     def score(self, images, grid_rows: int, grid_cols: int, want_logits: bool = False,
-              image_sets: Optional[Sequence[int]] = None, lane: int = 0, objectness: bool = False) -> ScoreResult:
+              image_sets: Optional[Sequence[int]] = None, lane: int = 0, objectness: bool = False, boxes: bool = True) -> ScoreResult:
         torch = self._torch
         if images.dtype != torch.uint8 or images.dim() != 4 or images.shape[-1] != 3 or not images.is_cuda:
             raise ValueError("score: images must be a cuda uint8 tensor [B,H,W,3]")
         if grid_rows < 1 or grid_cols < 1:
             raise ValueError("score: the grid must be at least 1x1")
+        if not boxes and grid_rows * grid_cols != 1:
+            raise ValueError("score: boxes=False needs a 1x1 grid (the cell of a detection is its box centre's)")
         images = images.contiguous()
         B, H, Wd, _ = images.shape
         dev = images.device
@@ -283,7 +285,7 @@
         r = ScoreResult(
             scores=torch.empty((B, npatch), dtype=torch.float32, device=dev),
             labels=torch.empty((B, npatch), dtype=torch.int32, device=dev),
-            boxes=torch.empty((B, npatch, 4), dtype=torch.float32, device=dev),
+            boxes=torch.empty((B, npatch, 4), dtype=torch.float32, device=dev) if boxes else None,
             cell_conf=torch.empty((B, ncell), dtype=torch.float64, device=dev),
             cell_mask=torch.empty((B, ncell), dtype=torch.int32, device=dev),
             n_kept=torch.empty((B,), dtype=torch.int32, device=dev),
@@ -300,13 +302,21 @@
             if len(qs) != 1:
                 raise ValueError("score: raw logits need the same query count for every image")
             r.logits = torch.empty((B, npatch, qs.pop()), dtype=torch.float32, device=dev)
-            r.boxes_cxcywh = torch.empty((B, npatch, 4), dtype=torch.float32, device=dev)
+            if boxes:
+                r.boxes_cxcywh = torch.empty((B, npatch, 4), dtype=torch.float32, device=dev)
         if objectness:
             if self.family != "owlv2":
                 raise ValueError("score: objectness needs an OWLv2 scorer (OWL-ViT has no objectness head)")
             r.objectness = torch.empty((B, npatch), dtype=torch.float32, device=dev)
         if self.family == "owlv2":
             self._prepare_v2(H, Wd)
+        if not boxes:
+            rc = self._lib.tstar_owl_score_cells(
+                self._h, int(lane), images.data_ptr(), B, H, Wd, grid_rows, grid_cols,
+                None if sets is None else sets.ctypes.data, r.scores.data_ptr(), r.labels.data_ptr(), r.cell_conf.data_ptr(),
+                r.cell_mask.data_ptr(), r.n_kept.data_ptr(), _lib.ptr(r.logits), _lib.ptr(r.objectness), _lib.stream_ptr())
+            _lib.check(rc, "tstar_owl_score_cells")
+            return r
         rc = self._lib.tstar_owl_score_lane_obj(
             self._h, int(lane), images.data_ptr(), B, H, Wd, grid_rows, grid_cols,
             None if sets is None else sets.ctypes.data, r.scores.data_ptr(), r.labels.data_ptr(), r.boxes.data_ptr(), r.cell_conf.data_ptr(),
```

Measured after the change: 12140, median of 6. 1.7% higher.
